# jkworldchampion/Video-Depth-Anything

Hardware: AMD Instinct MI355X
Metric: frames/sec at 1x32x518x518 fp16, ViT-L (higher is better)
Workload: dtype f16; 1 GPU; vitl fp16 32-frame clip forward, x=randn(1,32,3,518,518), seeded random weights (BASELINE.json configs[2]); parallelism=independent windows x1, world=1

## Files before the change

### video_depth_anything_amd/csrc/gemm.hip

```cpp
#include "gemm_epilogue.h"

namespace {
using vda_gemm::store_one;

constexpr int BK = 64;
constexpr int ROW_BYTES = BK * 2;
constexpr int NWAVES = 4;
constexpr int NTHREADS = NWAVES * 64;

template <int BM, int BN, int AMODE>
__global__ void __launch_bounds__(NTHREADS) gemm_kernel(const vda_gemm_args p) {
    constexpr int WTM = BM / 2, WTN = BN / 2;
    constexpr int MI = WTM / 16, NI = WTN / 16;
    constexpr int AJ = BM / 8 / NWAVES;
    constexpr int WJ = BN / 8 / NWAVES;
    constexpr int A_BYTES = BM * ROW_BYTES, W_BYTES = BN * ROW_BYTES, STAGE = A_BYTES + W_BYTES;

    extern __shared__ __attribute__((aligned(16))) char smem[];

    const int tid = threadIdx.x, lane = tid & 63;
    const int wave = __builtin_amdgcn_readfirstlane(tid >> 6);
    const int wm = wave >> 1, wn = wave & 1;

    const int nbn = (p.N + BN - 1) / BN;
    const int nwg = gridDim.x;
    const int bid = blockIdx.x;
    const int xcd = bid & 7, q = nwg >> 3, r = nwg & 7;
    const int t = (xcd < r ? xcd * (q + 1) : r * (q + 1) + (xcd - r) * q) + (bid >> 3);
    const int bm = t / nbn, bn = t - bm * nbn;
    const int m0 = bm * BM, n0 = bn * BN;

    const int lrow = lane >> 3;
    const int lchk = ((lane & 7) ^ lrow) * 8;
    const h16* a_src[AJ];
    int a_pix[AJ], a_iy0[AJ], a_ix0[AJ];
    const h16* w_src[WJ];
#pragma unroll
    for (int j = 0; j < AJ; ++j) {
        int m = m0 + (wave + NWAVES * j) * 8 + lrow;
        if constexpr (AMODE == VDA_A_DENSE) {
            m = min(m, p.M - 1);
            a_src[j] = (const h16*)p.A + (size_t)m * p.lda + lchk;
        } else {
            const bool ok = m < p.M;
            m = min(m, p.M - 1);
            const int hw = p.cHo * p.cWo;
            const int b = m / hw, rem = m - b * hw;
            const int oy = rem / p.cWo, ox = rem - oy * p.cWo;
            a_pix[j] = b * p.cH * p.cW;
            a_iy0[j] = ok ? oy * p.cStride - 1 : -100000;
            a_ix0[j] = ox * p.cStride - 1;
            a_src[j] = (const h16*)p.A + lchk;
        }
    }
#pragma unroll
    for (int j = 0; j < WJ; ++j) {
        const int n = min(n0 + (wave + NWAVES * j) * 8 + lrow, p.N - 1);
        w_src[j] = (const h16*)p.W + (size_t)n * p.K + lchk;
    }

    auto stage = [&](int kt, char* buf) {
        const int k0 = kt * BK;
        if constexpr (AMODE == VDA_A_DENSE) {
#pragma unroll
            for (int j = 0; j < AJ; ++j) glds16(a_src[j] + k0, buf + (wave + NWAVES * j) * 1024);
        } else {
            const int tap = k0 / p.cCin, ci0 = k0 - tap * p.cCin;
            const int ky = tap / 3, kx = tap - ky * 3;
#pragma unroll
            for (int j = 0; j < AJ; ++j) {
                const int iy = a_iy0[j] + ky, ix = a_ix0[j] + kx;
                const bool ok = (unsigned)iy < (unsigned)p.cH && (unsigned)ix < (unsigned)p.cW;
                const h16* src = ok ? a_src[j] + ((size_t)(a_pix[j] + iy * p.cW + ix) * p.cCin + ci0)
                                    : (const h16*)p.zero_page + lchk;
                glds16(src, buf + (wave + NWAVES * j) * 1024);
            }
        }
#pragma unroll
        for (int j = 0; j < WJ; ++j) glds16(w_src[j] + k0, buf + A_BYTES + (wave + NWAVES * j) * 1024);
    };

    f32x4 acc[MI][NI];
#pragma unroll
    for (int i = 0; i < MI; ++i)
#pragma unroll
        for (int j = 0; j < NI; ++j) acc[i][j] = f32x4{0.f, 0.f, 0.f, 0.f};

    const int frow = lane & 15, fchk = lane >> 4, fsw = lane & 7;
    const h16 relu_floor = p.relu_in ? (h16)0.f : (h16)(-65504.f);
    h16x8 relu_thr;
#pragma unroll
    for (int e = 0; e < 8; ++e) relu_thr[e] = relu_floor;

    auto compute = [&](const char* buf) {
        const char* At = buf + (wm * WTM + frow) * ROW_BYTES;
        const char* Wt = buf + A_BYTES + (wn * WTN + frow) * ROW_BYTES;
#pragma unroll
        for (int ks = 0; ks < 2; ++ks) {
            const int coff = ((ks * 4 + fchk) ^ fsw) << 4;
            h16x8 af[MI], wf[NI];
#pragma unroll
            for (int i = 0; i < MI; ++i) af[i] = *reinterpret_cast<const h16x8*>(At + i * 16 * ROW_BYTES + coff);
#pragma unroll
            for (int j = 0; j < NI; ++j) wf[j] = *reinterpret_cast<const h16x8*>(Wt + j * 16 * ROW_BYTES + coff);
            if constexpr (AMODE == VDA_A_CONV3X3) {
#pragma unroll
                for (int i = 0; i < MI; ++i) af[i] = __builtin_elementwise_max(af[i], relu_thr);
            }
#pragma unroll
            for (int i = 0; i < MI; ++i)
#pragma unroll
                for (int j = 0; j < NI; ++j)
                    acc[i][j] = __builtin_amdgcn_mfma_f32_16x16x32_f16(wf[j], af[i], acc[i][j], 0, 0, 0);
        }
    };

    const int nt = p.K / BK;
    stage(0, smem);
    asm volatile("s_waitcnt vmcnt(0)" ::: "memory");
    __syncthreads();
    int cur = 0;
    for (int kt = 0; kt < nt; ++kt) {
        if (kt + 1 < nt) stage(kt + 1, smem + (cur ^ 1) * STAGE);
        compute(smem + cur * STAGE);
        asm volatile("s_waitcnt vmcnt(0)" ::: "memory");
        __syncthreads();
        cur ^= 1;
    }

    const int em = m0 + wm * WTM + (lane & 15);
    const int en = n0 + wn * WTN + (lane >> 4) * 4;
    auto run = [&](auto epi_tag) {
        constexpr int EPI = decltype(epi_tag)::value;
        if constexpr (EPI == VDA_EPI_GEGLU_F16) {
#pragma unroll
            for (int i = 0; i < MI; ++i)
#pragma unroll
                for (int j = 0; j < NI; j += 2) store_one<EPI>(p, em + i * 16, en + j * 16, acc[i][j], acc[i][j + 1]);
        } else {
#pragma unroll
            for (int i = 0; i < MI; ++i)
#pragma unroll
                for (int j = 0; j < NI; ++j) store_one<EPI>(p, em + i * 16, en + j * 16, acc[i][j], acc[i][j]);
        }
    };
    vda_gemm::dispatch_epilogue(p.epilogue, run);
}

template <int BM, int BN, int AMODE>
int launch(const vda_gemm_args& a, hipStream_t s) {
    constexpr int smem = 2 * (BM + BN) * ROW_BYTES;
    static VdaKernelDeviceState dev_state;
    if (vda_prepare_kernel(reinterpret_cast<const void*>(&gemm_kernel<BM, BN, AMODE>), smem, dev_state) < 0) return 2;
    const int nbm = (a.M + BM - 1) / BM, nbn = (a.N + BN - 1) / BN;
    hipLaunchKernelGGL((gemm_kernel<BM, BN, AMODE>), dim3(nbm * nbn), dim3(NTHREADS), smem, s, a);
    VDA_LAUNCH_CHECK();
    return 0;
}

__global__ void __launch_bounds__(256) split_partials_kernel(const h16* __restrict__ hi, const h16* __restrict__ lo, float* __restrict__ part,
                                                             int M, int N, int ldc, int ld) {
    const int np = N >> 6;
    const long long i = (long long)blockIdx.x * 256 + threadIdx.x;
    if (i >= (long long)M * np) return;
    const int m = (int)(i / np), j = (int)(i - (long long)m * np);
    const h16* a = hi + (size_t)m * ldc + j * 64;
    const h16* b = lo + (size_t)m * ldc + j * 64;
    float sum = 0.f;
    for (int e = 0; e < 64; ++e) sum += (float)a[e] + (float)b[e];
    const float mean = sum * (1.f / 64.f);
    float sq = 0.f;
    for (int e = 0; e < 64; ++e) {
        const float d = ((float)a[e] + (float)b[e]) - mean;
        sq = fmaf(d, d, sq);
    }
    part[2 * ((size_t)j * ld + m)] = sum;
    part[2 * ((size_t)j * ld + m) + 1] = sq;
}

}

int vda_gemm256_dense_bn256(const vda_gemm_args& a, hipStream_t s);
int vda_gemm256_dense_bn128(const vda_gemm_args& a, hipStream_t s);
int vda_gemm256_conv_bn256(const vda_gemm_args& a, hipStream_t s);
int vda_gemm256_conv_bn128(const vda_gemm_args& a, hipStream_t s);
int vda_gemm256s_dense_bn256(const vda_gemm_args& a, hipStream_t s);
int vda_gemm256s_dense_bn128(const vda_gemm_args& a, hipStream_t s);
int vda_gemm256s_conv_bn256(const vda_gemm_args& a, hipStream_t s);
int vda_gemm256s_conv_bn128(const vda_gemm_args& a, hipStream_t s);
int vda_gemm256s_dense_bn128_bm192(const vda_gemm_args& a, hipStream_t s);
int vda_gemm256s_dense_bn128_bm192_x2(const vda_gemm_args& a, hipStream_t s);
int vda_gemm256s_dense_bn384_bm192(const vda_gemm_args& a, hipStream_t s);

int vda_gemm8p_dense_bn256(const vda_gemm_args& a, hipStream_t s);
int vda_gemm8p_conv_bn256(const vda_gemm_args& a, hipStream_t s);
int vda_gemm8p_dense_bn256_sched(const vda_gemm_args& a, hipStream_t s, int sched);
int vda_gemm8p_dense_bn128(const vda_gemm_args& a, hipStream_t s);
int vda_gemm8p_dense_bn256_bm192(const vda_gemm_args& a, hipStream_t s);
int vda_gemm8p_conv_bn128(const vda_gemm_args& a, hipStream_t s);

int vda_conv3x3_lds(const vda_gemm_args& a, hipStream_t s);

static int vda_gemm256s_launch(const vda_gemm_args& a, int bn, hipStream_t s) {
    if (a.a_mode == VDA_A_DENSE) return bn == 256 ? vda_gemm256s_dense_bn256(a, s) : vda_gemm256s_dense_bn128(a, s);
    return bn == 256 ? vda_gemm256s_conv_bn256(a, s) : vda_gemm256s_conv_bn128(a, s);
}

static int vda_gemm256_launch(const vda_gemm_args& a, int bn, hipStream_t s) {
    if (a.a_mode == VDA_A_DENSE) return bn == 256 ? vda_gemm256_dense_bn256(a, s) : vda_gemm256_dense_bn128(a, s);
    return bn == 256 ? vda_gemm256_conv_bn256(a, s) : vda_gemm256_conv_bn128(a, s);
}

static int launch_small(const vda_gemm_args& a, hipStream_t s) {
    const bool narrow = a.N <= 64;
    if (a.a_mode == VDA_A_DENSE) {
        const int rc = narrow ? launch<128, 64, VDA_A_DENSE>(a, s) : launch<128, 128, VDA_A_DENSE>(a, s);
        if (rc == 0 && a.epilogue == VDA_EPI_SCALE_RES_SPLIT) {
            const long long items = (long long)a.M * (a.N >> 6);
            hipLaunchKernelGGL(split_partials_kernel, dim3((unsigned)((items + 255) / 256)), dim3(256), 0, s, (const h16*)a.out, (const h16*)a.out2, a.stats, a.M,
                               a.N, a.ldc, a.stats_ld ? a.stats_ld : a.M);
            VDA_LAUNCH_CHECK();
        }
        return rc;
    }
    return narrow ? launch<128, 64, VDA_A_CONV3X3>(a, s) : launch<128, 128, VDA_A_CONV3X3>(a, s);
}

static int g_gemm_variant = -1;

static thread_local const char* g_last_kernel = "";

extern "C" const char* vda_gemm_last_kernel(void) { return g_last_kernel; }

extern "C" int vda_gemm_set_variant(int v) {
    g_gemm_variant = v;
    return 0;
}

static int g_gemm_debug = 0;

extern "C" int vda_gemm_set_debug(int flags) {
    g_gemm_debug = flags & 0xff;
    return 0;
}

static int device_cus() {
    static thread_local int ncu = 0;
    if (ncu == 0) {
        int dev = 0, cu = 0;
        (void)hipGetDevice(&dev);
        (void)hipDeviceGetAttribute(&cu, hipDeviceAttributeMultiprocessorCount, dev);
        ncu = cu < 8 ? 8 : (cu & ~7);
    }
    const int cap = g_vda_max_wgs;
    return (cap >= 8 && cap < ncu) ? (cap & ~7) : ncu;
}

static bool bm192_epilogue(int epilogue) {
    return epilogue == VDA_EPI_BIAS_F16 || epilogue == VDA_EPI_SCALE_RES_F32 || epilogue == VDA_EPI_SCALE_RES_SPLIT || epilogue == VDA_EPI_LN_BIAS_F16;
}

extern "C" int vda_gemm_plan_split(int M, int N, int K, int epilogue, int a_mode) {
    static const int allow = getenv("VDA_GEMM_SPLIT") ? atoi(getenv("VDA_GEMM_SPLIT")) : 1;
    static const int r192 = getenv("VDA_GEMM_R192") ? atoi(getenv("VDA_GEMM_R192")) : 84;
    if (!allow || a_mode != VDA_A_DENSE || !bm192_epilogue(epilogue) || M < 4096 || N < 256 || K < (allow == 2 ? 256 : 2048)) return M;
    const long long ncu = device_cus(), nbn = (N + 255) / 256;
    const long long rt = (M + 255) / 256;
    auto rounds = [&](long long tiles) { return (tiles + ncu - 1) / ncu; };
    const double t = 1.6 * (K / 64) + 5.0, launch = allow == 2 ? 0.0 : 10.0;
    const double single = (double)rounds(rt * nbn) * t;
    double best = single * 0.985;
    int best_m1 = M;
    for (long long r = 8; r * 256 < M; ++r) {
        const long long m2 = M - r * 256;
        if (m2 < 2048) break;
        const double cost = (double)rounds(r * nbn) * t + 0.01 * r192 * (double)rounds(((m2 + 191) / 192) * nbn) * t + launch;
        if (cost < best) {
            best = cost;
            best_m1 = (int)(r * 256);
        }
    }
    return best_m1;
}

static vda_gemm_args row_range(const vda_gemm_args& a0, int r0, int rows) {
    vda_gemm_args a = a0;
    if (a.lda == 0) a.lda = a.K;
    if (a.ldc == 0) a.ldc = a.N;
    vda_gemm_args p = a;
    auto adv = [&](const void* q, size_t bytes_per_row) -> const void* { return q ? (const char*)q + (size_t)r0 * bytes_per_row : nullptr; };
    const bool f32_out = a.epilogue == VDA_EPI_SCALE_RES_F32;
    const size_t ob = f32_out ? 4 : 2;
    p.A = adv(a.A, (size_t)a.lda * 2);
    p.out = const_cast<void*>(adv(a.out, (size_t)a.ldc * ob));
    if (a.epilogue == VDA_EPI_SCALE_RES_F32) p.res = adv(a.res, (size_t)a.ldc * 4);
    if (a.epilogue == VDA_EPI_SCALE_RES_SPLIT) {
        p.res = adv(a.res, (size_t)a.ldc * 2);
        p.res2 = adv(a.res2, (size_t)a.ldc * 2);
        p.out2 = const_cast<void*>(adv(a.out2, (size_t)a.ldc * 2));
        p.stats = (float*)const_cast<void*>(adv(a.stats, 8));
        p.stats_ld = a.stats_ld ? a.stats_ld : a.M;
        if (a.pos != nullptr && (const void*)a.pos != a.zero_page) p.pos = (const float*)adv(a.pos, 8);
    }
    if (a.epilogue == VDA_EPI_LN_BIAS_F16) p.stats = (float*)const_cast<void*>(adv(a.stats, 8));
    p.M = rows;
    return p;
}

extern "C" int vda_gemm_row_range(const vda_gemm_args* args, int r0, int rows, vda_gemm_args* out) {
    VDA_REQUIRE(args && out && r0 >= 0 && rows > 0 && r0 + rows <= args->M, "vda_gemm_row_range: bad range");
    VDA_REQUIRE(args->a_mode == VDA_A_DENSE && bm192_epilogue(args->epilogue), "vda_gemm_row_range: dense A and a row-splittable epilogue only");
    *out = row_range(*args, r0, rows);
    return 0;
}

static int vda_gemm_f16_impl(const vda_gemm_args* args, vda_stream_t stream, bool may_split);

extern "C" int vda_gemm_f16(const vda_gemm_args* args, vda_stream_t stream) { return vda_gemm_f16_impl(args, stream, true); }

static int vda_gemm_f16_impl(const vda_gemm_args* args, vda_stream_t stream, bool may_split) {
    VDA_REQUIRE(args != nullptr, "vda_gemm_f16: null args");
    vda_gemm_args a = *args;
    VDA_REQUIRE(a.A && a.W && a.out, "vda_gemm_f16: null operand");
    VDA_REQUIRE(a.M > 0 && a.N > 0 && a.K > 0, "vda_gemm_f16: empty problem M=%d N=%d K=%d", a.M, a.N, a.K);
    VDA_REQUIRE(a.K % BK == 0, "vda_gemm_f16: K=%d must be a multiple of %d (pad at pack time)", a.K, BK);
    VDA_REQUIRE(a.N % 4 == 0 && a.ldc % 4 == 0, "vda_gemm_f16: N=%d and ldc=%d must be multiples of 4", a.N, a.ldc);
    VDA_REQUIRE(((uintptr_t)a.A & 15) == 0 && ((uintptr_t)a.W & 15) == 0 && ((uintptr_t)a.out & 15) == 0,
                "vda_gemm_f16: operands must be 16-byte aligned");
    VDA_REQUIRE(a.epilogue >= 0 && a.epilogue <= VDA_EPI_LN_GELU_F16, "vda_gemm_f16: bad epilogue %d", a.epilogue);
    if (a.a_mode == VDA_A_DENSE) {
        VDA_REQUIRE(a.relu_in == 0, "vda_gemm_f16: relu_in is only built for the conv A operand");
        VDA_REQUIRE((a.lda >= a.K || a.lda == 0) && a.lda % 8 == 0, "vda_gemm_f16: lda=%d must be >= K (or 0 = broadcast row) and a multiple of 8", a.lda);
    } else if (a.a_mode == VDA_A_CONV3X3) {
        VDA_REQUIRE(a.zero_page != nullptr, "vda_gemm_f16: conv needs zero_page");
        VDA_REQUIRE(a.cCin % BK == 0 && a.K == 9 * a.cCin, "vda_gemm_f16: conv needs Cin%%64==0 and K==9*Cin (Cin=%d K=%d)", a.cCin, a.K);
        VDA_REQUIRE(a.cStride == 1 || a.cStride == 2, "vda_gemm_f16: conv stride %d", a.cStride);
        VDA_REQUIRE(a.cHo == (a.cH + 2 - 3) / a.cStride + 1 && a.cWo == (a.cW + 2 - 3) / a.cStride + 1,
                    "vda_gemm_f16: conv output size mismatch");
        VDA_REQUIRE(a.M == a.cB * a.cHo * a.cWo, "vda_gemm_f16: conv M=%d != B*Ho*Wo", a.M);
        VDA_REQUIRE((long long)a.cB * a.cH * a.cW * a.cCin < (1ll << 31), "vda_gemm_f16: conv input too large for 32-bit pixel index");
    } else {
        VDA_REQUIRE(false, "vda_gemm_f16: bad a_mode %d", a.a_mode);
    }
    switch (a.epilogue) {
        case VDA_EPI_SCALE_RES_F32:
        case VDA_EPI_SCALE_RES_F32_H:
        case VDA_EPI_RES_F16:
            VDA_REQUIRE(a.res != nullptr, "vda_gemm_f16: residual epilogue needs res");
            break;
        case VDA_EPI_GEGLU_F16:
            VDA_REQUIRE(a.N % 32 == 0, "vda_gemm_f16: GEGLU needs N%%32==0");
            break;
        case VDA_EPI_SCALE_RES_SPLIT:
            VDA_REQUIRE(a.res != nullptr && a.res2 != nullptr && a.out2 != nullptr && a.stats != nullptr,
                        "vda_gemm_f16: the split-residual epilogue needs res, res2 (hi / lo planes), out2 and stats");
            VDA_REQUIRE(a.N % 64 == 0 && a.ldc % 8 == 0 && a.a_mode == VDA_A_DENSE, "vda_gemm_f16: the split-residual epilogue needs a dense A operand, N%%64==0 and ldc%%8==0");
            VDA_REQUIRE(((uintptr_t)a.res & 15) == 0 && ((uintptr_t)a.res2 & 15) == 0 && ((uintptr_t)a.out2 & 15) == 0 && ((uintptr_t)a.stats & 7) == 0,
                        "vda_gemm_f16: split-residual planes must be 16-byte aligned");
            if (a.pos != nullptr && (const void*)a.pos != a.zero_page) {
                VDA_REQUIRE(((uintptr_t)a.pos & 7) == 0, "vda_gemm_f16: pos (re-centring statistics) must be 8-byte aligned");
                a.P = 2;
            } else {
                VDA_REQUIRE(a.zero_page != nullptr, "vda_gemm_f16: the split-residual epilogue without pos needs zero_page");
                a.pos = (const float*)a.zero_page;
                a.P = 0;
            }
            break;
        case VDA_EPI_LN_BIAS_F16:
        case VDA_EPI_LN_GELU_F16:
            VDA_REQUIRE(a.stats != nullptr && a.gamma != nullptr && a.bias != nullptr && a.a_mode == VDA_A_DENSE,
                        "vda_gemm_f16: a LayerNorm-folded epilogue needs a dense A operand, stats (mean, rstd rows), gamma (= c1) and bias (= c2)");
            VDA_REQUIRE(((uintptr_t)a.stats & 7) == 0, "vda_gemm_f16: stats must be 8-byte aligned");
            break;
        case VDA_EPI_PATCH_F32:
            VDA_REQUIRE(a.pos != nullptr && a.P > 0 && a.M % a.P == 0, "vda_gemm_f16: patch epilogue needs pos and M%%P==0");
            break;
        case VDA_EPI_CONVT_F16:
            VDA_REQUIRE(a.tK > 0 && a.tCout > 0 && a.tCout % 4 == 0 && a.N == a.tK * a.tK * a.tCout && a.M % (a.tH * a.tW) == 0,
                        "vda_gemm_f16: bad ConvTranspose geometry");
            break;
        default:
            break;
    }
    hipStream_t s = (hipStream_t)stream;
    static const int conv_lds = getenv("VDA_CONV_LDS") ? atoi(getenv("VDA_CONV_LDS")) : 1;
    if (a.a_mode == VDA_A_CONV3X3 && ((g_gemm_variant < 0 && conv_lds) || g_gemm_variant == 7)) {
        const int rc = vda_conv3x3_lds(a, s);
        if (rc >= 0) {
            g_last_kernel = a.N <= 32 ? "conv3x3_lds_kernel<1>" : "conv3x3_lds_kernel<2>";
            return rc;
        }
    }
    const bool fits32 = (a.a_mode == VDA_A_DENSE ? (long long)a.M * a.lda : 0ll) + a.K < (1ll << 31) && (long long)a.N * a.K < (1ll << 31);
    VDA_REQUIRE(fits32 || g_gemm_variant == 0 || g_gemm_variant < 0, "vda_gemm_f16: operand too large for the 256-row kernel's 32-bit offsets");
    if (!fits32) return launch_small(a, s);
    int big = 0, small_mfma = 1;
    bool eight = g_gemm_variant >= 5 && (g_gemm_variant & 15) == 5;
    if (eight) big = 256;
    if (g_gemm_variant == 1 || g_gemm_variant == 3) big = 256;
    if (g_gemm_variant == 2 || g_gemm_variant == 4 || g_gemm_variant == 8 || g_gemm_variant == 10 || g_gemm_variant == 11) big = 128;
    if (g_gemm_variant == 1 || g_gemm_variant == 2) small_mfma = 0;
    if (g_gemm_variant == 9) {
        eight = true;
        big = 128;
    }
    static const int big_min_n = getenv("VDA_GEMM_BIG_MIN_N") ? atoi(getenv("VDA_GEMM_BIG_MIN_N")) : 192;
    if (g_gemm_variant < 0 && a.N >= big_min_n && a.M >= 2048) {
        const int pad256 = (a.N + 255) / 256 * 256, pad128 = (a.N + 127) / 128 * 128;
        big = pad128 < pad256 ? 128 : 256;
        static const int eight128 = getenv("VDA_GEMM_8P128") ? atoi(getenv("VDA_GEMM_8P128")) : 0;
        if (big == 256 || eight128) eight = true;
    }
    if (big && (a.N % 8 != 0 || a.ldc % 8 != 0)) {
        VDA_REQUIRE(g_gemm_variant < 0, "vda_gemm_f16: the 256-row kernel needs N and ldc to be multiples of 8");
        big = 0;
    }
    if (big) {
        vda_gemm_args a8 = a;
        static const int stagger = getenv("VDA_GEMM_STAGGER") ? atoi(getenv("VDA_GEMM_STAGGER")) : 0;
        if (!stagger) a8.relu_in |= 16 << 8;
        if (stagger == 2) a8.relu_in |= 32 << 8;
        if (eight && g_gemm_variant > 0) a8.relu_in = (a.relu_in & 0xff) | (((g_gemm_variant >> 4) & 0xff) << 8);
        a8.relu_in |= g_gemm_debug << 16;
        static const long long nt_mb = getenv("VDA_GEMM_NT_MB") ? atoll(getenv("VDA_GEMM_NT_MB")) : 192;
        if (nt_mb > 0 && (long long)a.M * a.N * 2 >= nt_mb * 1000000ll) a8.relu_in |= 1 << 24;
        const int sched8 = (eight && g_gemm_variant > 0) ? ((g_gemm_variant >> 5) & 3) : 0;
        bool tall192 = g_gemm_variant == 8 && a.a_mode == VDA_A_DENSE;
        const int ncu = device_cus();
        if (g_gemm_variant < 0 && !eight && big == 128 && a.a_mode == VDA_A_DENSE) {
            const long long nbn = (a.N + 127) / 128;
            const long long r256 = (((a.M + 255) / 256) * nbn + ncu - 1) / ncu, r192 = (((a.M + 191) / 192) * nbn + ncu - 1) / ncu;
            static const int allow192 = getenv("VDA_GEMM_BM192") ? atoi(getenv("VDA_GEMM_BM192")) : 1;
            tall192 = allow192 && r192 * 3 * 100 < r256 * 4 * 85;
        }
        static const int small_grid = getenv("VDA_GEMM_SMALL_GRID") ? atoi(getenv("VDA_GEMM_SMALL_GRID")) : 1;
        if (g_gemm_variant < 0 && small_grid && ((long long)(a.M + 255) / 256) * ((a.N + big - 1) / big) * 2 <= ncu) {
            g_last_kernel = a.a_mode == VDA_A_DENSE ? (a.N <= 64 ? "gemm_kernel<128, 64, 0>" : "gemm_kernel<128, 128, 0>")
                                                    : (a.N <= 64 ? "gemm_kernel<128, 64, 1>" : "gemm_kernel<128, 128, 1>");
            return launch_small(a, s);
        }
        static const int wide384 = getenv("VDA_GEMM_BN384") ? atoi(getenv("VDA_GEMM_BN384")) : 2;
        const bool ln_epi = a.epilogue == VDA_EPI_LN_BIAS_F16 || a.epilogue == VDA_EPI_LN_GELU_F16;
        const bool auto384 = g_gemm_variant < 0 && a.tile_rows == 0 &&
                             (wide384 == 1 ? (!eight && a.N <= 1152)
                                            : wide384 == 2 ? ((a.N == 384 && a.K >= 1024) || (ln_epi && a.N <= 1536))
                                            : wide384 == 3 ? (a.N == 384 && a.K >= 1024)
                                            : wide384 == 4 ? ((a.N == 384 && a.K >= 1024) || (ln_epi && a.N == 1536)) : false);
        if (a.a_mode == VDA_A_DENSE && a.N % 384 == 0 && (auto384 || g_gemm_variant == 10)) {
            const int rc384 = vda_gemm256s_dense_bn384_bm192(a8, s);
            if (rc384 >= 0) {
                static thread_local char name384[64];
                snprintf(name384, sizeof(name384), "gemm256s_kernel<384, %d, %d, 192, 1>", a.a_mode, a.epilogue);
                g_last_kernel = name384;
                return rc384;
            }
        }
        if (eight && big == 256 && a.a_mode == VDA_A_DENSE && g_gemm_variant < 0 && may_split && a.tile_rows == 0 && a.sched == nullptr && a.lda != 0) {
            const int m1 = vda_gemm_plan_split(a.M, a.N, a.K, a.epilogue, a.a_mode);
            if (m1 < a.M) {
                vda_gemm_args p1 = row_range(a, 0, m1), p2 = row_range(a, m1, a.M - m1);
                p2.tile_rows = 192;
                const int rc1 = vda_gemm_f16_impl(&p1, stream, false);
                if (rc1 != 0) return rc1;
                return vda_gemm_f16_impl(&p2, stream, false);
            }
        }
        if (eight && big == 256 && a.a_mode == VDA_A_DENSE && (a.tile_rows == 192 || g_gemm_variant == 5 + 16 * 64)) {
            const int rc192 = vda_gemm8p_dense_bn256_bm192(a8, s);
            if (rc192 >= 0) {
                static thread_local char name192[64];
                snprintf(name192, sizeof(name192), "gemm8p_kernel<256, %d, %d, 1, 192, %s>", a.a_mode, a.epilogue, a.sched ? "true" : "false");
                g_last_kernel = name192;
                return rc192;
            }
        }
        if (g_gemm_variant == 11 && a.a_mode == VDA_A_DENSE) {
            const int rcx2 = vda_gemm256s_dense_bn128_bm192_x2(a8, s);
            if (rcx2 >= 0) {
                static thread_local char namex2[64];
                snprintf(namex2, sizeof(namex2), "gemm256s_kernel<128, %d, %d, 192, 2>", a.a_mode, a.epilogue);
                g_last_kernel = namex2;
                return rcx2;
            }
        }
        if (tall192) {
            const int rc192 = vda_gemm256s_dense_bn128_bm192(a8, s);
            if (rc192 >= 0) {
                static thread_local char name192[64];
                snprintf(name192, sizeof(name192), "gemm256s_kernel<128, %d, %d, 192, 1>", a.a_mode, a.epilogue);
                g_last_kernel = name192;
                return rc192;
            }
        }
        const int rc = !eight ? (small_mfma ? vda_gemm256s_launch(a8, big, s) : vda_gemm256_launch(a, big, s))
                       : big == 128 ? (a.a_mode == VDA_A_DENSE ? vda_gemm8p_dense_bn128(a8, s) : vda_gemm8p_conv_bn128(a8, s))
                       : a.a_mode == VDA_A_DENSE ? (sched8 ? vda_gemm8p_dense_bn256_sched(a8, s, sched8) : vda_gemm8p_dense_bn256(a8, s))
                                                 : vda_gemm8p_conv_bn256(a8, s);
        if (rc >= 0) {
            static thread_local char name[64];
            const int sch = sched8 == 1 ? 0 : sched8 == 2 ? 2 : 1;
            if (eight) snprintf(name, sizeof(name), "gemm8p_kernel<%d, %d, %d, %d, 256, %s>", big, a.a_mode, a.epilogue, sch, (a.sched && sch == 1) ? "true" : "false");
            else if (small_mfma) snprintf(name, sizeof(name), "gemm256s_kernel<%d, %d, %d, 256, 1>", big, a.a_mode, a.epilogue);
            else snprintf(name, sizeof(name), "gemm256_kernel<%d, %d, %d>", big, a.a_mode, a.epilogue);
            g_last_kernel = name;
            return rc;
        }
    }
    g_last_kernel = a.a_mode == VDA_A_DENSE ? (a.N <= 64 ? "gemm_kernel<128, 64, 0>" : "gemm_kernel<128, 128, 0>")
                                            : (a.N <= 64 ? "gemm_kernel<128, 64, 1>" : "gemm_kernel<128, 128, 1>");
    return launch_small(a, s);
}
```

### video_depth_anything_amd/csrc/host.hip

```cpp
#include "vda_common.h"
#include <string.h>
#include <exception>
#include <type_traits>
#include <array>
#include <map>
#include <string>
#include <vector>

namespace {

constexpr int PATCH = 14, POS_GRID = 37, KPATCH = 640, GN_GROUPS = 32, TEMPORAL_HEADS = 8;
constexpr float ENC_LN_EPS = 1e-6f, GN_EPS = 1e-6f, TMP_LN_EPS = 1e-5f;

inline int pad64(int c) { return (c + 63) / 64 * 64; }

#define VDA_TRY(expr)            \
    do {                         \
        const int rc_ = (expr);  \
        if (rc_ != 0) return rc_; \
    } while (0)

#define VDA_HIP(expr)                                                      \
    do {                                                                   \
        const hipError_t e_ = (expr);                                      \
        if (e_ != hipSuccess) {                                            \
            vda_set_error("%s: %s", #expr, hipGetErrorString(e_));         \
            return 2;                                                      \
        }                                                                  \
    } while (0)

template <typename T>
__global__ void pack_matrix_kernel(const float* __restrict__ src, T* __restrict__ dst, int N, int K, int Npad, int Kpad) {
    const size_t total = (size_t)Npad * Kpad;
    for (size_t i = (size_t)blockIdx.x * 256 + threadIdx.x; i < total; i += (size_t)gridDim.x * 256) {
        const int n = (int)(i / Kpad), k = (int)(i - (size_t)n * Kpad);
        dst[i] = (n < N && k < K) ? (T)src[(size_t)n * K + k] : (T)0.f;
    }
}
template <typename T>
__global__ void pack_conv3x3_kernel(const float* __restrict__ src, T* __restrict__ dst, int Co, int Ci, int Copad, int Cipad) {
    const size_t total = (size_t)Copad * 9 * Cipad;
    for (size_t i = (size_t)blockIdx.x * 256 + threadIdx.x; i < total; i += (size_t)gridDim.x * 256) {
        const int ci = (int)(i % Cipad);
        const size_t t = i / Cipad;
        const int tap = (int)(t % 9), co = (int)(t / 9);
        dst[i] = (co < Co && ci < Ci) ? (T)src[((size_t)co * Ci + ci) * 9 + tap] : (T)0.f;
    }
}
template <typename T>
__global__ void pack_convt_kernel(const float* __restrict__ src, T* __restrict__ dst, int Ci, int Co, int k, int cpad) {
    const size_t total = (size_t)k * k * cpad * cpad;
    for (size_t i = (size_t)blockIdx.x * 256 + threadIdx.x; i < total; i += (size_t)gridDim.x * 256) {
        const int ci = (int)(i % cpad);
        const size_t t = i / cpad;
        const int co = (int)(t % cpad), tap = (int)(t / cpad);
        dst[i] = (co < Co && ci < Ci) ? (T)src[((size_t)ci * Co + co) * k * k + tap] : (T)0.f;
    }
}
__global__ void expand_convt_bias_kernel(const float* __restrict__ b, float* __restrict__ dst, int Co, int kk, int cpad) {
    const int i = blockIdx.x * 256 + threadIdx.x;
    if (i >= kk * cpad) return;
    const int co = i % cpad;
    dst[i] = co < Co ? b[co] : 0.f;
}
template <typename T>
__global__ void pack_geglu_kernel(const float* __restrict__ src, T* __restrict__ dst, int n, int K) {
    const size_t total = (size_t)2 * n * K;
    for (size_t i = (size_t)blockIdx.x * 256 + threadIdx.x; i < total; i += (size_t)gridDim.x * 256) {
        const int R = (int)(i / K), k = (int)(i - (size_t)R * K);
        const int blk = R >> 5, within = R & 31;
        const int srow = within < 16 ? blk * 16 + within : n + blk * 16 + (within - 16);
        dst[i] = (T)src[(size_t)srow * K + k];
    }
}

inline unsigned grid_for(size_t items) {
    const size_t b = (items + 255) / 256;
    return (unsigned)(b < 1 ? 1 : (b > 65535 ? 65535 : b));
}

#ifndef VDA_LN_FOLD_DEFAULT
#define VDA_LN_FOLD_DEFAULT 1
#endif

__global__ void __launch_bounds__(256) poison_on_overflow_kernel(const int* __restrict__ flag, float* __restrict__ depth, long long n,
                                                                 volatile int* __restrict__ host_report) {
    if (*flag == 0) return;
    for (long long i = (long long)blockIdx.x * 256 + threadIdx.x; i < n; i += (long long)gridDim.x * 256) depth[i] = __builtin_nanf("");
    if (blockIdx.x == 0 && threadIdx.x == 0) {
        *host_report = 1;
        __threadfence_system();
    }
}

struct Raw {
    float* d = nullptr;
    std::vector<int64_t> dims;
    size_t n = 0;
};

struct ProfSample {
    std::string name;
    double flops;
    hipEvent_t e0, e1;
};
struct Profile {
    int every = 0;
    double min_flops = 0.0;
    std::map<std::array<int, 5>, int> seen;
    std::map<std::string, std::pair<long long, double>> launches;
    std::vector<ProfSample> samples;
};

struct Layout {
    int gemm_launches = 0;
    std::map<std::string, std::pair<size_t, size_t>> bufs;
    std::vector<std::string> order;
    size_t total = 0;
};

}

struct vda_model {
    vda_config cfg;
    int device = 0;
    std::map<std::string, std::vector<int64_t>> spec;
    std::map<std::string, Raw> raw;
    std::map<std::string, void*> mat[2];
    std::map<std::string, float*> vec;
    bool finalized = false, packed[2] = {false, false};
    float oc3_bias = 0.f;
    void* zero_page = nullptr;
    std::map<std::pair<int, int>, float*> pos_cache;
    void* ws = nullptr;
    int64_t ws_bytes = 0;
    bool ws_owned = false;
    std::map<std::array<int, 5>, Layout> layouts;
    std::vector<void*> owned;
    int ocp[4] = {0, 0, 0, 0}, Fhp = 0;
    std::array<int, 5> last_key = {0, 0, 0, 0, -1};
    Profile prof;
    int residual_in_ln = 0;
    int dyn_sched = 0;
    int ln_fold = VDA_LN_FOLD_DEFAULT;
    int oc1_fused = 1;
    int head_overlap = 0;
    struct Side {
        hipStream_t stream = nullptr;
        hipEvent_t fork = nullptr, join = nullptr;
    };
    std::map<hipStream_t, Side> sides;
    int mlp_fused = 0;
    volatile int32_t* ovf_host = nullptr;
};

namespace {

using Spec = std::map<std::string, std::vector<int64_t>>;

void build_spec(const vda_config& c, Spec& s) {
    const int64_t D = c.embed_dim, F = c.features;
    const int64_t oc[4] = {c.out_channels[0], c.out_channels[1], c.out_channels[2], c.out_channels[3]};
    auto put = [&](const std::string& k, std::vector<int64_t> v) { s[k] = std::move(v); };
    const std::string p = "pretrained.";
    put(p + "cls_token", {1, 1, D});
    put(p + "pos_embed", {1, POS_GRID * POS_GRID + 1, D});
    put(p + "mask_token", {1, D});
    put(p + "patch_embed.proj.weight", {D, 3, PATCH, PATCH});
    put(p + "patch_embed.proj.bias", {D});
    for (int i = 0; i < c.depth; ++i) {
        const std::string b = p + "blocks." + std::to_string(i) + ".";
        put(b + "norm1.weight", {D});
        put(b + "norm1.bias", {D});
        put(b + "attn.qkv.weight", {3 * D, D});
        put(b + "attn.qkv.bias", {3 * D});
        put(b + "attn.proj.weight", {D, D});
        put(b + "attn.proj.bias", {D});
        put(b + "ls1.gamma", {D});
        put(b + "norm2.weight", {D});
        put(b + "norm2.bias", {D});
        put(b + "mlp.fc1.weight", {4 * D, D});
        put(b + "mlp.fc1.bias", {4 * D});
        put(b + "mlp.fc2.weight", {D, 4 * D});
        put(b + "mlp.fc2.bias", {D});
        put(b + "ls2.gamma", {D});
    }
    put(p + "norm.weight", {D});
    put(p + "norm.bias", {D});
    const std::string h = "head.";
    for (int i = 0; i < 4; ++i) {
        put(h + "projects." + std::to_string(i) + ".weight", {oc[i], D, 1, 1});
        put(h + "projects." + std::to_string(i) + ".bias", {oc[i]});
    }
    put(h + "resize_layers.0.weight", {oc[0], oc[0], 4, 4});
    put(h + "resize_layers.0.bias", {oc[0]});
    put(h + "resize_layers.1.weight", {oc[1], oc[1], 2, 2});
    put(h + "resize_layers.1.bias", {oc[1]});
    put(h + "resize_layers.3.weight", {oc[3], oc[3], 3, 3});
    put(h + "resize_layers.3.bias", {oc[3]});
    if (c.use_clstoken)
        for (int i = 0; i < 4; ++i) {
            put(h + "readout_projects." + std::to_string(i) + ".0.weight", {D, 2 * D});
            put(h + "readout_projects." + std::to_string(i) + ".0.bias", {D});
        }
    const std::string sc = h + "scratch.";
    for (int i = 0; i < 4; ++i) put(sc + "layer" + std::to_string(i + 1) + "_rn.weight", {F, oc[i], 3, 3});
    for (int i = 1; i <= 4; ++i) {
        const std::string r = sc + "refinenet" + std::to_string(i) + ".";
        put(r + "out_conv.weight", {F, F, 1, 1});
        put(r + "out_conv.bias", {F});
        for (int u = 1; u <= 2; ++u)
            for (int cc = 1; cc <= 2; ++cc) {
                const std::string k = r + "resConfUnit" + std::to_string(u) + ".conv" + std::to_string(cc);
                put(k + ".weight", {F, F, 3, 3});
                put(k + ".bias", {F});
            }
        if (c.use_bn)
            for (int u = 1; u <= 2; ++u)
                for (int cc = 1; cc <= 2; ++cc) {
                    const std::string k = r + "resConfUnit" + std::to_string(u) + ".bn" + std::to_string(cc) + ".";
                    put(k + "weight", {F});
                    put(k + "bias", {F});
                    put(k + "running_mean", {F});
                    put(k + "running_var", {F});
                    put(k + "num_batches_tracked", {});
                }
    }
    put(sc + "output_conv1.weight", {F / 2, F, 3, 3});
    put(sc + "output_conv1.bias", {F / 2});
    put(sc + "output_conv2.0.weight", {32, F / 2, 3, 3});
    put(sc + "output_conv2.0.bias", {32});
    put(sc + "output_conv2.2.weight", {1, 32, 1, 1});
    put(sc + "output_conv2.2.bias", {1});
    const int64_t tc[4] = {oc[2], oc[3], F, F};
    for (int m = 0; m < 4; ++m) {
        const int64_t C = tc[m];
        const std::string t = h + "motion_modules." + std::to_string(m) + ".temporal_transformer.";
        put(t + "norm.weight", {C});
        put(t + "norm.bias", {C});
        put(t + "proj_in.weight", {C, C});
        put(t + "proj_in.bias", {C});
        const std::string tb = t + "transformer_blocks.0.";
        for (int a = 0; a < 2; ++a) {
            const std::string ab = tb + "attention_blocks." + std::to_string(a) + ".";
            put(ab + "to_q.weight", {C, C});
            put(ab + "to_k.weight", {C, C});
            put(ab + "to_v.weight", {C, C});
            put(ab + "to_out.0.weight", {C, C});
            put(ab + "to_out.0.bias", {C});
            if (!c.pe_rope) put(ab + "pos_encoder.pe", {1, c.num_frames, C});
            put(tb + "norms." + std::to_string(a) + ".weight", {C});
            put(tb + "norms." + std::to_string(a) + ".bias", {C});
        }
        put(tb + "ff.net.0.proj.weight", {8 * C, C});
        put(tb + "ff.net.0.proj.bias", {8 * C});
        put(tb + "ff.net.2.weight", {C, 4 * C});
        put(tb + "ff.net.2.bias", {C});
        put(tb + "ff_norm.weight", {C});
        put(tb + "ff_norm.bias", {C});
        put(t + "proj_out.weight", {C, C});
        put(t + "proj_out.bias", {C});
    }
}

int dev_alloc(vda_model* h, size_t bytes, void** out) {
    void* p = nullptr;
    VDA_HIP(hipMalloc(&p, bytes < 256 ? 256 : bytes));
    h->owned.push_back(p);
    *out = p;
    return 0;
}

int require_device(const vda_model* h, const char* what) {
    int dev = -1;
    VDA_HIP(hipGetDevice(&dev));
    if (dev != h->device) {
        vda_set_error("%s: the handle lives on device %d but device %d is current (one handle per device; make it current)", what, h->device, dev);
        return 1;
    }
    return 0;
}

__global__ void __launch_bounds__(256) fold_bn_kernel(const float* __restrict__ W, const float* __restrict__ b, const float* __restrict__ g,
                                                      const float* __restrict__ beta, const float* __restrict__ rm, const float* __restrict__ rv,
                                                      float* __restrict__ Wo, float* __restrict__ bo, int Co, int per_co) {
    const long long n = (long long)Co * per_co;
    for (long long i = (long long)blockIdx.x * 256 + threadIdx.x; i < n; i += (long long)gridDim.x * 256) {
        const int co = (int)(i / per_co);
        const float sc = g[co] / sqrtf(rv[co] + 1e-5f);
        Wo[i] = W[i] * sc;
        if (i - (long long)co * per_co == 0) bo[co] = (b[co] - rm[co]) * sc + beta[co];
    }
}

template <typename T>
int pack_all(vda_model* h, int prec) {
    const vda_config& c = h->cfg;
    hipStream_t s = nullptr;
    auto raw = [&](const std::string& k) -> const float* { return h->raw.at(k).d; };
    auto mat = [&](const std::string& key, size_t elems, T** out) -> int {
        void* p = nullptr;
        VDA_TRY(dev_alloc(h, elems * sizeof(T), &p));
        h->mat[prec][key] = p;
        *out = (T*)p;
        return 0;
    };
    auto lin = [&](const std::string& key, const std::string& name, int N, int K, int Npad, int Kpad) -> int {
        T* d = nullptr;
        VDA_TRY(mat(key, (size_t)Npad * Kpad, &d));
        hipLaunchKernelGGL((pack_matrix_kernel<T>), dim3(grid_for((size_t)Npad * Kpad)), dim3(256), 0, s, raw(name), d, N, K, Npad, Kpad);
        return 0;
    };
    auto conv = [&](const std::string& key, const std::string& name, int Co, int Ci, int Copad, int Cipad) -> int {
        T* d = nullptr;
        VDA_TRY(mat(key, (size_t)Copad * 9 * Cipad, &d));
        hipLaunchKernelGGL((pack_conv3x3_kernel<T>), dim3(grid_for((size_t)Copad * 9 * Cipad)), dim3(256), 0, s, raw(name), d, Co, Ci, Copad, Cipad);
        return 0;
    };
    const bool vecs = h->vec.empty();
    auto vecp = [&](const std::string& key, const std::string& name, int n, int npad) -> int {
        if (!vecs) return 0;
        void* p = nullptr;
        VDA_TRY(dev_alloc(h, (size_t)npad * sizeof(float), &p));
        h->vec[key] = (float*)p;
        hipLaunchKernelGGL((pack_matrix_kernel<float>), dim3(grid_for(npad)), dim3(256), 0, s, raw(name), (float*)p, 1, n, 1, npad);
        return 0;
    };
    const int D = c.embed_dim, Fe = c.features;
    const int* oc = c.out_channels;
    const int* ocp = h->ocp;
    const int Fh = Fe / 2, Fhp = h->Fhp;
    const std::string p = "pretrained.";
    VDA_TRY(lin("patch.w", p + "patch_embed.proj.weight", D, 588, D, KPATCH));
    VDA_TRY(vecp("patch.b", p + "patch_embed.proj.bias", D, D));
    VDA_TRY(vecp("cls", p + "cls_token", D, D));
    for (int i = 0; i < c.depth; ++i) {
        const std::string b = p + "blocks." + std::to_string(i) + ".", k = "b" + std::to_string(i) + ".";
        VDA_TRY(vecp(k + "norm1.weight", b + "norm1.weight", D, D));
        VDA_TRY(vecp(k + "norm1.bias", b + "norm1.bias", D, D));
        VDA_TRY(vecp(k + "norm2.weight", b + "norm2.weight", D, D));
        VDA_TRY(vecp(k + "norm2.bias", b + "norm2.bias", D, D));
        VDA_TRY(vecp(k + "attn.qkv.bias", b + "attn.qkv.bias", 3 * D, 3 * D));
        VDA_TRY(vecp(k + "attn.proj.bias", b + "attn.proj.bias", D, D));
        VDA_TRY(vecp(k + "mlp.fc1.bias", b + "mlp.fc1.bias", 4 * D, 4 * D));
        VDA_TRY(vecp(k + "mlp.fc2.bias", b + "mlp.fc2.bias", D, D));
        VDA_TRY(vecp(k + "ls1.gamma", b + "ls1.gamma", D, D));
        VDA_TRY(vecp(k + "ls2.gamma", b + "ls2.gamma", D, D));
        VDA_TRY(lin(k + "attn.qkv.weight", b + "attn.qkv.weight", 3 * D, D, 3 * D, D));
        VDA_TRY(lin(k + "attn.proj.weight", b + "attn.proj.weight", D, D, D, D));
        VDA_TRY(lin(k + "mlp.fc1.weight", b + "mlp.fc1.weight", 4 * D, D, 4 * D, D));
        VDA_TRY(lin(k + "mlp.fc2.weight", b + "mlp.fc2.weight", D, 4 * D, D, 4 * D));
        if constexpr (std::is_same<T, h16>::value) {
            const char* pairs[2][3] = {{"attn.qkv", "norm1", nullptr}, {"mlp.fc1", "norm2", nullptr}};
            const int outs[2] = {3 * D, 4 * D};
            for (int j = 0; j < 2; ++j) {
                const std::string lk = pairs[j][0], nk = pairs[j][1];
                T* d = nullptr;
                VDA_TRY(mat(k + lk + ".weight.ln", (size_t)outs[j] * D, &d));
                void *c1 = nullptr, *c2 = nullptr;
                VDA_TRY(dev_alloc(h, (size_t)outs[j] * sizeof(float), &c1));
                VDA_TRY(dev_alloc(h, (size_t)outs[j] * sizeof(float), &c2));
                h->vec[k + lk + ".c1"] = (float*)c1;
                h->vec[k + lk + ".c2"] = (float*)c2;
                VDA_TRY(vda_fold_ln_weight(raw(b + lk + ".weight"), raw(b + lk + ".bias"), raw(b + nk + ".weight"), raw(b + nk + ".bias"), d, (float*)c1,
                                           (float*)c2, outs[j], D, s));
            }
            if (vda_mlp_fused_supported(D, 4 * D)) {
                T* d = nullptr;
                VDA_TRY(mat(k + "mlp.fc2.weight.perm", (size_t)D * 4 * D, &d));
                VDA_TRY(vda_mlp_permute_w2_f16(h->mat[prec].at(k + "mlp.fc2.weight"), d, D, 4 * D, s));
            }
        }
    }
    VDA_TRY(vecp("norm.w", p + "norm.weight", D, D));
    VDA_TRY(vecp("norm.b", p + "norm.bias", D, D));
    const std::string hd = "head.";
    if (c.use_clstoken)
        for (int i = 0; i < 4; ++i) {
            const std::string n = hd + "readout_projects." + std::to_string(i) + ".0", k = "readout" + std::to_string(i);
            VDA_TRY(lin(k + ".w", n + ".weight", D, 2 * D, D, 2 * D));
            VDA_TRY(vecp(k + ".b", n + ".bias", D, D));
        }
    for (int i = 0; i < 4; ++i) {
        const std::string n = hd + "projects." + std::to_string(i), k = "proj" + std::to_string(i);
        VDA_TRY(lin(k + ".w", n + ".weight", oc[i], D, ocp[i], D));
        VDA_TRY(vecp(k + ".b", n + ".bias", oc[i], ocp[i]));
    }
    for (int i = 0; i < 2; ++i) {
        const int kk = i == 0 ? 4 : 2, cp = ocp[i];
        const std::string n = hd + "resize_layers." + std::to_string(i), k = "resize" + std::to_string(i);
        T* d = nullptr;
        VDA_TRY(mat(k + ".w", (size_t)kk * kk * cp * cp, &d));
        hipLaunchKernelGGL((pack_convt_kernel<T>), dim3(grid_for((size_t)kk * kk * cp * cp)), dim3(256), 0, s, raw(n + ".weight"), d, oc[i], oc[i], kk, cp);
        if (vecs) {
            void* bp = nullptr;
            VDA_TRY(dev_alloc(h, (size_t)kk * kk * cp * sizeof(float), &bp));
            h->vec[k + ".b"] = (float*)bp;
            hipLaunchKernelGGL(expand_convt_bias_kernel, dim3((kk * kk * cp + 255) / 256), dim3(256), 0, s, raw(n + ".bias"), (float*)bp, oc[i], kk * kk, cp);
        }
    }
    VDA_TRY(conv("resize3.w", hd + "resize_layers.3.weight", oc[3], oc[3], ocp[3], ocp[3]));
    VDA_TRY(vecp("resize3.b", hd + "resize_layers.3.bias", oc[3], ocp[3]));
    const std::string sc = hd + "scratch.";
    for (int i = 0; i < 4; ++i)
        VDA_TRY(conv("rn" + std::to_string(i + 1) + ".w", sc + "layer" + std::to_string(i + 1) + "_rn.weight", Fe, oc[i], Fe, ocp[i]));
    for (int i = 1; i <= 4; ++i) {
        const std::string r = sc + "refinenet" + std::to_string(i) + ".", k = "ref" + std::to_string(i) + ".";
        VDA_TRY(lin(k + "out.w", r + "out_conv.weight", Fe, Fe, Fe, Fe));
        VDA_TRY(vecp(k + "out.b", r + "out_conv.bias", Fe, Fe));
        for (int u = 1; u <= 2; ++u)
            for (int cc = 1; cc <= 2; ++cc) {
                const std::string rn = r + "resConfUnit" + std::to_string(u) + ".conv" + std::to_string(cc);
                const std::string kn = k + "rcu" + std::to_string(u) + ".c" + std::to_string(cc);
                if (c.use_bn) {
                    const std::string bn = r + "resConfUnit" + std::to_string(u) + ".bn" + std::to_string(cc) + ".";
                    Raw& fw = h->raw[rn + ".weight.bn"];
                    Raw& fb = h->raw[rn + ".bias.bn"];
                    if (fw.d == nullptr) {
                        void *pw = nullptr, *pb = nullptr;
                        VDA_TRY(dev_alloc(h, (size_t)Fe * Fe * 9 * sizeof(float), &pw));
                        VDA_TRY(dev_alloc(h, (size_t)Fe * sizeof(float), &pb));
                        fw.d = (float*)pw, fw.n = (size_t)Fe * Fe * 9;
                        fb.d = (float*)pb, fb.n = Fe;
                    }
                    hipLaunchKernelGGL(fold_bn_kernel, dim3(grid_for((size_t)Fe * Fe * 9)), dim3(256), 0, s, raw(rn + ".weight"), raw(rn + ".bias"), raw(bn + "weight"),
                                       raw(bn + "bias"), raw(bn + "running_mean"), raw(bn + "running_var"), fw.d, fb.d, Fe, Fe * 9);
                    VDA_TRY(conv(kn + ".w", rn + ".weight.bn", Fe, Fe, Fe, Fe));
                    VDA_TRY(vecp(kn + ".b", rn + ".bias.bn", Fe, Fe));
                    continue;
                }
                VDA_TRY(conv(kn + ".w", rn + ".weight", Fe, Fe, Fe, Fe));
                VDA_TRY(vecp(kn + ".b", rn + ".bias", Fe, Fe));
            }
    }
    VDA_TRY(conv("oc1.w", sc + "output_conv1.weight", Fh, Fe, Fhp, Fe));
    VDA_TRY(vecp("oc1.b", sc + "output_conv1.bias", Fh, Fhp));
    VDA_TRY(conv("oc2.w", sc + "output_conv2.0.weight", 32, Fh, 32, Fhp));
    VDA_TRY(vecp("oc2.b", sc + "output_conv2.0.bias", 32, 32));
    VDA_TRY(vecp("oc3.w", sc + "output_conv2.2.weight", 32, 32));
    const int tc[4] = {ocp[2], ocp[3], Fe, Fe};
    for (int m = 0; m < 4; ++m) {
        const int Cc = tc[m];
        const std::string t = hd + "motion_modules." + std::to_string(m) + ".temporal_transformer.", k = "tm" + std::to_string(m) + ".";
        VDA_TRY(vecp(k + "gn.w", t + "norm.weight", Cc, Cc));
        VDA_TRY(vecp(k + "gn.b", t + "norm.bias", Cc, Cc));
        VDA_TRY(lin(k + "in.w", t + "proj_in.weight", Cc, Cc, Cc, Cc));
        VDA_TRY(vecp(k + "in.b", t + "proj_in.bias", Cc, Cc));
        VDA_TRY(lin(k + "out.w", t + "proj_out.weight", Cc, Cc, Cc, Cc));
        VDA_TRY(vecp(k + "out.b", t + "proj_out.bias", Cc, Cc));
        const std::string tb = t + "transformer_blocks.0.";
        for (int a = 0; a < 2; ++a) {
            const std::string ab = tb + "attention_blocks." + std::to_string(a) + ".", ka = k + "a" + std::to_string(a) + ".";
            T* d = nullptr;
            VDA_TRY(mat(ka + "qkv.w", (size_t)3 * Cc * Cc, &d));
            const char* names[3] = {"to_q.weight", "to_k.weight", "to_v.weight"};
            for (int j = 0; j < 3; ++j)
                hipLaunchKernelGGL((pack_matrix_kernel<T>), dim3(grid_for((size_t)Cc * Cc)), dim3(256), 0, s, raw(ab + names[j]),
                                   d + (size_t)j * Cc * Cc, Cc, Cc, Cc, Cc);
            VDA_TRY(lin(ka + "out.w", ab + "to_out.0.weight", Cc, Cc, Cc, Cc));
            VDA_TRY(vecp(ka + "out.b", ab + "to_out.0.bias", Cc, Cc));
            if (!c.pe_rope) VDA_TRY(vecp(ka + "pe", ab + "pos_encoder.pe", c.num_frames * Cc, c.num_frames * Cc));
            VDA_TRY(vecp(ka + "ln.w", tb + "norms." + std::to_string(a) + ".weight", Cc, Cc));
            VDA_TRY(vecp(ka + "ln.b", tb + "norms." + std::to_string(a) + ".bias", Cc, Cc));
        }
        VDA_TRY(vecp(k + "ffln.w", tb + "ff_norm.weight", Cc, Cc));
        VDA_TRY(vecp(k + "ffln.b", tb + "ff_norm.bias", Cc, Cc));
        {
            T* d = nullptr;
            VDA_TRY(mat(k + "ff1.w", (size_t)8 * Cc * Cc, &d));
            hipLaunchKernelGGL((pack_geglu_kernel<T>), dim3(grid_for((size_t)8 * Cc * Cc)), dim3(256), 0, s, raw(tb + "ff.net.0.proj.weight"), d, 4 * Cc, Cc);
            if (vecs) {
                void* bp = nullptr;
                VDA_TRY(dev_alloc(h, (size_t)8 * Cc * sizeof(float), &bp));
                h->vec[k + "ff1.b"] = (float*)bp;
                hipLaunchKernelGGL((pack_geglu_kernel<float>), dim3(grid_for((size_t)8 * Cc)), dim3(256), 0, s, raw(tb + "ff.net.0.proj.bias"), (float*)bp, 4 * Cc, 1);
            }
        }
        VDA_TRY(lin(k + "ff2.w", tb + "ff.net.2.weight", Cc, 4 * Cc, Cc, 4 * Cc));
        VDA_TRY(vecp(k + "ff2.b", tb + "ff.net.2.bias", Cc, Cc));
    }
    VDA_HIP(hipGetLastError());
    VDA_HIP(hipStreamSynchronize(s));
    h->packed[prec] = true;
    return 0;
}

struct Run {
    vda_model* h;
    int prec;
    bool dry;
    Layout* lay;
    hipStream_t s;
    size_t ab;
    int32_t* sched = nullptr;
    int nsched = 0;

    void* buf(const std::string& name, size_t elems, size_t esize) {
        const size_t bytes = (elems * esize + 255) & ~(size_t)255;
        if (dry) {
            auto it = lay->bufs.find(name);
            if (it == lay->bufs.end()) {
                lay->bufs[name] = {0, bytes};
                lay->order.push_back(name);
            } else if (it->second.second < bytes) {
                it->second.second = bytes;
            }
            return (void*)(uintptr_t)256;
        }
        return (char*)h->ws + lay->bufs.at(name).first;
    }
    void* act(const std::string& name, size_t elems) { return buf(name, elems, ab); }
    float* f32(const std::string& name, size_t elems) { return (float*)buf(name, elems, 4); }
    const void* W(const std::string& k) const { return dry ? nullptr : h->mat[prec].at(k); }
    const float* V(const std::string& k) const { return dry ? nullptr : h->vec.at(k); }

    int gemm(vda_gemm_args a) {
        if (prec == VDA_PREC_F16) {
            const int m1 = vda_gemm_plan_split(a.M, a.N, a.K, a.epilogue, a.a_mode);
            if (m1 < a.M) {
                if (dry) {
                    VDA_TRY(gemm_one(a));
                    return gemm_one(a);
                }
                vda_gemm_args p1, p2;
                a.zero_page = h->zero_page;
                VDA_TRY(vda_gemm_row_range(&a, 0, m1, &p1));
                VDA_TRY(vda_gemm_row_range(&a, m1, a.M - m1, &p2));
                p1.tile_rows = 256;
                p2.tile_rows = 192;
                VDA_TRY(gemm_one(p1));
                return gemm_one(p2);
            }
        }
        return gemm_one(a);
    }
    int gemm_one(vda_gemm_args a) {
        if (prec == VDA_PREC_F16 && h->dyn_sched) {
            if (!dry && sched != nullptr) a.sched = sched + 8 * nsched;
            ++nsched;
        }
        if (dry) return 0;
        a.zero_page = h->zero_page;
        if (a.lda == 0) a.lda = a.K;
        if (a.ldc == 0) a.ldc = a.N;
        Profile& pf = h->prof;
        if (pf.every <= 0) return prec == VDA_PREC_F32 ? vda_gemm_f32(&a, s) : vda_gemm_f16(&a, s);
        const std::array<int, 5> key = {a.M, a.N, a.K, a.epilogue, a.a_mode};
        const int n = pf.seen[key]++;
        const bool timed = n % pf.every == 0 && 2.0 * a.M * a.N * a.K >= pf.min_flops;
        ProfSample smp;
        if (timed) {
            VDA_HIP(hipEventCreate(&smp.e0));
            VDA_HIP(hipEventCreate(&smp.e1));
            VDA_HIP(hipEventRecord(smp.e0, s));
        }
        VDA_TRY(prec == VDA_PREC_F32 ? vda_gemm_f32(&a, s) : vda_gemm_f16(&a, s));
        const std::string name = prec == VDA_PREC_F32 ? std::string("gemm_f32_kernel") : std::string(vda_gemm_last_kernel());
        const double flops = 2.0 * a.M * a.N * a.K;
        auto& tot = pf.launches[name];
        tot.first += 1;
        tot.second += flops;
        if (timed) {
            VDA_HIP(hipEventRecord(smp.e1, s));
            smp.name = name;
            smp.flops = flops;
            pf.samples.push_back(smp);
        }
        return 0;
    }
    int dense(const void* A, const void* Wm, void* out, int epi, int M, int N, int K, const float* bias = nullptr, const void* res = nullptr,
              const float* gamma = nullptr, int ldc = 0) {
        vda_gemm_args a = {};
        a.A = A, a.W = Wm, a.out = out, a.bias = bias, a.res = res, a.gamma = gamma;
        a.M = M, a.N = N, a.K = K, a.ldc = ldc, a.a_mode = VDA_A_DENSE, a.epilogue = epi;
        return gemm(a);
    }
    int conv3x3(const void* x, const std::string& wname, void* out, int B, int H, int Wd, int Cin, int Cout, int epi, int stride,
                const float* bias, bool relu_in = false, const void* res = nullptr, const void* res2 = nullptr) {
        const int Ho = (H - 1) / stride + 1, Wo = (Wd - 1) / stride + 1;
        vda_gemm_args a = {};
        a.A = x, a.W = W(wname), a.out = out, a.bias = bias, a.res = res, a.res2 = res2;
        a.M = B * Ho * Wo, a.N = Cout, a.K = 9 * Cin, a.a_mode = VDA_A_CONV3X3, a.epilogue = epi, a.relu_in = relu_in ? 1 : 0;
        a.cB = B, a.cH = H, a.cW = Wd, a.cCin = Cin, a.cHo = Ho, a.cWo = Wo, a.cStride = stride;
        return gemm(a);
    }
    int layernorm(const float* x, void* out, const float* w, const float* b, float eps, int rows, int D, int group = 0, int skip = 0,
                  const float* pe = nullptr, int pe_rows = 0, int pe_steps = 0) {
        if (dry) return 0;
        return prec == VDA_PREC_F32 ? vda_layernorm_f32_f32(x, (float*)out, w, b, eps, rows, D, group, skip, pe, pe_rows, pe_steps, s)
                                    : vda_layernorm_f32_f16(x, out, w, b, eps, rows, D, group, skip, pe, pe_rows, pe_steps, s);
    }
    int bilinear(const void* x, void* out, int B, int hh, int ww, int H, int Wd, int C) {
        if (dry) return 0;
        return prec == VDA_PREC_F32 ? vda_bilinear_nhwc_f32((const float*)x, (float*)out, nullptr, B, hh, ww, H, Wd, C, s)
                                    : vda_bilinear_nhwc_f16(x, out, nullptr, B, hh, ww, H, Wd, C, s);
    }

    int temporal(int m, const void* x, int B, int T, int hw, int Cc, const std::string& tag, void** result) {
        const std::string k = "tm" + std::to_string(m) + ".";
        const int BT = B * T, rows = BT * hw;
        int chunks = (hw + 31) / 32;
        chunks = chunks < 1 ? 1 : (chunks > 16 ? 16 : chunks);
        float* part = f32("gn_partial", (size_t)BT * chunks * GN_GROUPS * 2);
        void* g = act("tm_g", (size_t)rows * Cc);
        if (!dry)
            VDA_TRY(prec == VDA_PREC_F32 ? vda_groupnorm_nhwc_f32((const float*)x, (float*)g, V(k + "gn.w"), V(k + "gn.b"), GN_EPS, BT, hw, Cc, GN_GROUPS, part, chunks, s)
                                         : vda_groupnorm_nhwc_f16(x, g, V(k + "gn.w"), V(k + "gn.b"), GN_EPS, BT, hw, Cc, GN_GROUPS, part, chunks, s));
        float* hs = f32("tm_hs", (size_t)rows * Cc);
        VDA_TRY(dense(g, W(k + "in.w"), hs, VDA_EPI_BIAS_F32, rows, Cc, Cc, V(k + "in.b")));
        void* n = act("tm_n", (size_t)rows * Cc);
        void* qkv = act("tm_qkv", (size_t)rows * 3 * Cc);
        void* ao = act("tm_ao", (size_t)rows * Cc);
        for (int a = 0; a < 2; ++a) {
            const std::string ka = k + "a" + std::to_string(a) + ".";
            const bool rope = h->cfg.pe_rope != 0;
            VDA_TRY(layernorm(hs, n, V(ka + "ln.w"), V(ka + "ln.b"), TMP_LN_EPS, rows, Cc, 0, 0, rope ? nullptr : V(ka + "pe"), hw, T));
            VDA_TRY(dense(n, W(ka + "qkv.w"), qkv, VDA_EPI_BIAS_F16, rows, 3 * Cc, Cc));
            for (int b = 0; b < B && !dry; ++b) {
                const size_t r0 = (size_t)b * T * hw;
                if (rope)
                    VDA_TRY(prec == VDA_PREC_F32 ? vda_rope_qk_f32((float*)qkv + r0 * 3 * Cc, T, hw, Cc, s) : vda_rope_qk_f16((h16*)qkv + r0 * 3 * Cc, T, hw, Cc, s));
                VDA_TRY(prec == VDA_PREC_F32
                            ? vda_temporal_attention_f32((const float*)qkv + r0 * 3 * Cc, (float*)ao + r0 * Cc, T, hw, Cc, TEMPORAL_HEADS, s)
                            : vda_temporal_attention_f16((const h16*)qkv + r0 * 3 * Cc, (h16*)ao + r0 * Cc, T, hw, Cc, TEMPORAL_HEADS, s));
            }
            VDA_TRY(dense(ao, W(ka + "out.w"), hs, VDA_EPI_SCALE_RES_F32, rows, Cc, Cc, V(ka + "out.b"), hs));
        }
        VDA_TRY(layernorm(hs, n, V(k + "ffln.w"), V(k + "ffln.b"), TMP_LN_EPS, rows, Cc));
        void* gg = act("tm_gg", (size_t)rows * 4 * Cc);
        VDA_TRY(dense(n, W(k + "ff1.w"), gg, VDA_EPI_GEGLU_F16, rows, 8 * Cc, Cc, V(k + "ff1.b"), nullptr, nullptr, 4 * Cc));
        void* hh = act("tm_hh", (size_t)rows * Cc);
        VDA_TRY(dense(gg, W(k + "ff2.w"), hh, VDA_EPI_SCALE_RES_F32_H, rows, Cc, 4 * Cc, V(k + "ff2.b"), hs));
        void* out = act(tag, (size_t)rows * Cc);
        VDA_TRY(dense(hh, W(k + "out.w"), out, VDA_EPI_RES_F16, rows, Cc, Cc, V(k + "out.b"), x));
        *result = out;
        return 0;
    }

    int rcu(int i, int u, const void* x, void* out, int B, int H, int Wd, int Fe, const void* res2 = nullptr) {
        const std::string k = "ref" + std::to_string(i) + ".rcu" + std::to_string(u) + ".";
        void* y = act("rcu_y", (size_t)B * H * Wd * Fe);
        VDA_TRY(conv3x3(x, k + "c1.w", y, B, H, Wd, Fe, Fe, VDA_EPI_BIAS_RELU_F16, 1, V(k + "c1.b"), true));
        VDA_TRY(conv3x3(y, k + "c2.w", out, B, H, Wd, Fe, Fe, VDA_EPI_RES_F16, 1, V(k + "c2.b"), false, x, res2));
        return 0;
    }
    int fusion(int i, const void* x0, const void* x1, int B, int H, int Wd, int Ho, int Wo, int Fe, const std::string& tag, void** result,
               bool upsample = true) {
        const size_t rows = (size_t)B * H * Wd;
        const void* sm = x0;
        if (x1 != nullptr) {
            void* t = act("fus_s", rows * Fe);
            VDA_TRY(rcu(i, 1, x1, t, B, H, Wd, Fe, x0));
            sm = t;
        }
        void* r = act("fus_r", rows * Fe);
        VDA_TRY(rcu(i, 2, sm, r, B, H, Wd, Fe));
        void* c = act(upsample ? "fus_c" : tag, rows * Fe);
        const std::string k = "ref" + std::to_string(i) + ".out.";
        VDA_TRY(dense(r, W(k + "w"), c, VDA_EPI_BIAS_F16, (int)rows, Fe, Fe, V(k + "b")));
        if (!upsample) {
            *result = c;
            return 0;
        }
        void* out = act(tag, (size_t)B * Ho * Wo * Fe);
        VDA_TRY(bilinear(c, out, B, H, Wd, Ho, Wo, Fe));
        *result = out;
        return 0;
    }

    int forward(const float* x, float* depth, int B, int T, int H, int Wd) {
        const vda_config& c = h->cfg;
        const int BT = B * T, ph = H / PATCH, pw = Wd / PATCH;
        const int P = ph * pw, D = c.embed_dim, NH = c.num_heads, Nt = P + 1, rows = BT * Nt;
        if (prec == VDA_PREC_F16 && h->dyn_sched) {
            const int cap = dry ? 4096 : lay->gemm_launches;
            sched = (int32_t*)buf("sched", (size_t)8 * (cap > 0 ? cap : 1), 4);
            if (!dry) VDA_HIP(hipMemsetAsync(sched, 0, (size_t)32 * lay->gemm_launches, s));
            nsched = 0;
        }
        void* a0 = act("a0", (size_t)BT * P * KPATCH);
        if (!dry) {
            VDA_HIP(hipMemsetAsync(a0, 0, (size_t)BT * P * KPATCH * ab, s));
            VDA_TRY(prec == VDA_PREC_F32 ? vda_patchify_f32_f32(x, (float*)a0, BT, H, Wd, KPATCH, s) : vda_patchify_f32_f16(x, a0, BT, H, Wd, KPATCH, s));
        }
        float* tok = f32("tok", (size_t)rows * D);
        const float* pos = dry ? nullptr : h->pos_cache.at({H, Wd});
        {
            vda_gemm_args a = {};
            a.A = a0, a.W = W("patch.w"), a.out = tok, a.bias = V("patch.b"), a.pos = pos;
            a.M = BT * P, a.N = D, a.K = KPATCH, a.a_mode = VDA_A_DENSE, a.epilogue = VDA_EPI_PATCH_F32, a.P = P;
            VDA_TRY(gemm(a));
        }
        if (!dry) VDA_TRY(vda_cls_rows_f32(tok, V("cls"), pos, BT, P, D, s));
        void* xn = act("xn", (size_t)rows * D);
        void* qkv = act("qkv", (size_t)rows * 3 * D);
        void* ao = act("ao", (size_t)rows * D);
        void* hid = nullptr;
        void* taps[4] = {nullptr, nullptr, nullptr, nullptr};
        int ntap = 0;
        const bool defer = prec == VDA_PREC_F16 && h->residual_in_ln != 0;
        const bool fold = prec == VDA_PREC_F16 && h->ln_fold != 0 && !defer && D % 64 == 0;
        const bool mlp1 = fold && h->mlp_fused != 0 && vda_mlp_fused_supported(D, 4 * D) != 0;
        if (!mlp1) hid = act("hid", (size_t)rows * 4 * D);
        void* thi = fold ? buf("tok_hi", (size_t)rows * D, 2) : nullptr;
        void* tlo = fold ? buf("tok_lo", (size_t)rows * D, 2) : nullptr;
        float* lnpart = fold ? f32("ln_part", (size_t)rows * (D / 64) * 2) : nullptr;
        float* lnstat = fold ? f32("ln_stat", (size_t)rows * 2) : nullptr;
        int32_t* ovf = fold ? (int32_t*)buf("overflow", 1, 4) : nullptr;
        if (fold && !dry) VDA_HIP(hipMemsetAsync(ovf, 0, 4, s));
        if (fold && !dry) VDA_TRY(vda_split_center_stats_f32(tok, thi, tlo, lnstat, ENC_LN_EPS, rows, D, s));
        auto ln_gemm = [&](const std::string& wk, void* out, int epi, int N) -> int {
            vda_gemm_args a = {};
            a.A = thi, a.W = W(wk + ".weight.ln"), a.out = out, a.bias = V(wk + ".c2"), a.gamma = V(wk + ".c1"), a.stats = lnstat;
            a.M = rows, a.N = N, a.K = D, a.a_mode = VDA_A_DENSE, a.epilogue = epi;
            return gemm(a);
        };
        auto res_gemm = [&](const void* A, const std::string& wk, const std::string& gk, int K, bool stats_next) -> int {
            vda_gemm_args a = {};
            a.A = A, a.W = W(wk + ".weight"), a.out = thi, a.out2 = tlo, a.res = thi, a.res2 = tlo, a.bias = V(wk + ".bias"), a.gamma = V(gk);
            a.stats = lnpart;
            a.pos = lnstat;
            a.M = rows, a.N = D, a.K = K, a.a_mode = VDA_A_DENSE, a.epilogue = VDA_EPI_SCALE_RES_SPLIT;
            VDA_TRY(gemm(a));
            (void)stats_next;
            if (!dry) VDA_TRY(vda_ln_stats_finalize(lnpart, lnstat, ENC_LN_EPS, rows, D / 64, ovf, s));
            return 0;
        };
        auto tap_ln = [&](void* out, int group, int skip) -> int {
            if (dry) return 0;
            return fold ? vda_layernorm_split_f16(thi, tlo, out, V("norm.w"), V("norm.b"), ENC_LN_EPS, rows, D, group, skip, s)
                        : vda_layernorm_f32_f16(tok, out, V("norm.w"), V("norm.b"), ENC_LN_EPS, rows, D, group, skip, nullptr, 0, 0, s);
        };
        void* yb = defer ? act("ybuf", (size_t)rows * D) : nullptr;
        auto ln_res = [&](const float* gamma, void* out, const float* w, const float* b, int group, int skip) -> int {
            if (dry) return 0;
            return vda_layernorm_residual_f32_f16(tok, yb, gamma, out, w, b, ENC_LN_EPS, rows, D, group, skip, s);
        };
        bool xn_ready = false;
        const int* ocp = h->ocp;
        const int Fe = c.features, Fhp = h->Fhp;
        const int h1 = 4 * ph, w1 = 4 * pw, h2 = 2 * ph, w2 = 2 * pw, h4 = (ph - 1) / 2 + 1, w4 = (pw - 1) / 2 + 1;
        void *l1r = nullptr, *l2r = nullptr, *l3r = nullptr;
        auto head_early = [&]() -> int {
            void* t0 = act("t0", (size_t)BT * P * ocp[0]);
            VDA_TRY(dense(taps[0], W("proj0.w"), t0, VDA_EPI_BIAS_F16, BT * P, ocp[0], D, V("proj0.b")));
            void* l1 = act("l1", (size_t)BT * h1 * w1 * ocp[0]);
            {
                vda_gemm_args a = {};
                a.A = t0, a.W = W("resize0.w"), a.out = l1, a.bias = V("resize0.b");
                a.M = BT * P, a.N = 16 * ocp[0], a.K = ocp[0], a.ldc = ocp[0], a.a_mode = VDA_A_DENSE, a.epilogue = VDA_EPI_CONVT_F16;
                a.tK = 4, a.tH = ph, a.tW = pw, a.tCout = ocp[0];
                VDA_TRY(gemm(a));
            }
            void* t1 = act("t1", (size_t)BT * P * ocp[1]);
            VDA_TRY(dense(taps[1], W("proj1.w"), t1, VDA_EPI_BIAS_F16, BT * P, ocp[1], D, V("proj1.b")));
            void* l2 = act("l2", (size_t)BT * h2 * w2 * ocp[1]);
            {
                vda_gemm_args a = {};
                a.A = t1, a.W = W("resize1.w"), a.out = l2, a.bias = V("resize1.b");
                a.M = BT * P, a.N = 4 * ocp[1], a.K = ocp[1], a.ldc = ocp[1], a.a_mode = VDA_A_DENSE, a.epilogue = VDA_EPI_CONVT_F16;
                a.tK = 2, a.tH = ph, a.tW = pw, a.tCout = ocp[1];
                VDA_TRY(gemm(a));
            }
            void* l3 = act("l3", (size_t)BT * P * ocp[2]);
            VDA_TRY(dense(taps[2], W("proj2.w"), l3, VDA_EPI_BIAS_F16, BT * P, ocp[2], D, V("proj2.b")));
            void* l3t = nullptr;
            VDA_TRY(temporal(0, l3, B, T, P, ocp[2], "l3t", &l3t));
            l1r = act("l1r", (size_t)BT * h1 * w1 * Fe);
            VDA_TRY(conv3x3(l1, "rn1.w", l1r, BT, h1, w1, ocp[0], Fe, VDA_EPI_BIAS_F16, 1, nullptr));
            l2r = act("l2r", (size_t)BT * h2 * w2 * Fe);
            VDA_TRY(conv3x3(l2, "rn2.w", l2r, BT, h2, w2, ocp[1], Fe, VDA_EPI_BIAS_F16, 1, nullptr));
            l3r = act("l3r", (size_t)BT * P * Fe);
            VDA_TRY(conv3x3(l3t, "rn3.w", l3r, BT, ph, pw, ocp[2], Fe, VDA_EPI_BIAS_F16, 1, nullptr));
            return 0;
        };
        bool early_done = false;
        vda_model::Side* side = nullptr;
        for (int i = 0; i < c.depth; ++i) {
            const std::string k = "b" + std::to_string(i) + ".";
            if (fold) {
                VDA_TRY(ln_gemm(k + "attn.qkv", qkv, VDA_EPI_LN_BIAS_F16, 3 * D));
            } else {
                if (!xn_ready) VDA_TRY(layernorm(tok, xn, V(k + "norm1.weight"), V(k + "norm1.bias"), ENC_LN_EPS, rows, D));
                xn_ready = false;
                VDA_TRY(dense(xn, W(k + "attn.qkv.weight"), qkv, VDA_EPI_BIAS_F16, rows, 3 * D, D, V(k + "attn.qkv.bias")));
            }
            if (!dry) VDA_TRY(prec == VDA_PREC_F32 ? vda_attention_f32((const float*)qkv, (float*)ao, BT, Nt, NH, s) : vda_attention_f16(qkv, ao, BT, Nt, NH, s));
            if (fold) {
                VDA_TRY(res_gemm(ao, k + "attn.proj", k + "ls1.gamma", D, true));
            } else if (defer) {
                VDA_TRY(dense(ao, W(k + "attn.proj.weight"), yb, VDA_EPI_BIAS_F16, rows, D, D, V(k + "attn.proj.bias")));
                VDA_TRY(ln_res(V(k + "ls1.gamma"), xn, V(k + "norm2.weight"), V(k + "norm2.bias"), 0, 0));
            } else {
                VDA_TRY(dense(ao, W(k + "attn.proj.weight"), tok, VDA_EPI_SCALE_RES_F32, rows, D, D, V(k + "attn.proj.bias"), tok, V(k + "ls1.gamma")));
                VDA_TRY(layernorm(tok, xn, V(k + "norm2.weight"), V(k + "norm2.bias"), ENC_LN_EPS, rows, D));
            }
            if (mlp1) {
                if (!dry)
                    VDA_TRY(vda_mlp_fused_f16(thi, lnstat, W(k + "mlp.fc1.weight.ln"), V(k + "mlp.fc1.c1"), V(k + "mlp.fc1.c2"), W(k + "mlp.fc2.weight.perm"),
                                              V(k + "mlp.fc2.bias"), V(k + "ls2.gamma"), thi, tlo, lnpart, rows, D, 4 * D, rows, s));
            } else if (fold) VDA_TRY(ln_gemm(k + "mlp.fc1", hid, VDA_EPI_LN_GELU_F16, 4 * D));
            else VDA_TRY(dense(xn, W(k + "mlp.fc1.weight"), hid, VDA_EPI_BIAS_GELU_F16, rows, 4 * D, D, V(k + "mlp.fc1.bias")));
            bool is_tap = false;
            for (int t = 0; t < 4; ++t) is_tap = is_tap || c.taps[t] == i;
            const bool last = i + 1 == c.depth;
            void* tp = (is_tap && ntap < 4) ? act("tap" + std::to_string(ntap), (size_t)BT * P * D) : nullptr;
            if (fold) {
                if (mlp1) {
                    if (!dry) VDA_TRY(vda_ln_stats_finalize(lnpart, lnstat, ENC_LN_EPS, rows, D / 64, ovf, s));
                } else {
                    VDA_TRY(res_gemm(hid, k + "mlp.fc2", k + "ls2.gamma", 4 * D, !last));
                }
                if (tp != nullptr) VDA_TRY(tap_ln(tp, Nt, 1));
            } else if (defer) {
                VDA_TRY(dense(hid, W(k + "mlp.fc2.weight"), yb, VDA_EPI_BIAS_F16, rows, D, 4 * D, V(k + "mlp.fc2.bias")));
                if (last && tp != nullptr) {
                    VDA_TRY(ln_res(V(k + "ls2.gamma"), tp, V("norm.w"), V("norm.b"), Nt, 1));
                } else {
                    const std::string kn = "b" + std::to_string(last ? i : i + 1) + ".";
                    VDA_TRY(ln_res(V(k + "ls2.gamma"), xn, V(kn + "norm1.weight"), V(kn + "norm1.bias"), 0, 0));
                    xn_ready = true;
                    if (tp != nullptr) VDA_TRY(layernorm(tok, tp, V("norm.w"), V("norm.b"), ENC_LN_EPS, rows, D, Nt, 1));
                }
            } else {
                VDA_TRY(dense(hid, W(k + "mlp.fc2.weight"), tok, VDA_EPI_SCALE_RES_F32, rows, D, 4 * D, V(k + "mlp.fc2.bias"), tok, V(k + "ls2.gamma")));
                if (tp != nullptr) VDA_TRY(layernorm(tok, tp, V("norm.w"), V("norm.b"), ENC_LN_EPS, rows, D, Nt, 1));
            }
            if (tp != nullptr) {
                if (c.use_clstoken) {
                    void* full = act("rd_full", (size_t)rows * D);
                    VDA_TRY(fold ? tap_ln(full, 0, 0) : layernorm(tok, full, V("norm.w"), V("norm.b"), ENC_LN_EPS, rows, D));
                    void* cat = act("rd_cat", (size_t)BT * P * 2 * D);
                    if (!dry)
                        VDA_TRY(prec == VDA_PREC_F32 ? vda_readout_concat_f32((const float*)full, (float*)cat, BT, P, D, s)
                                                     : vda_readout_concat_f16(full, cat, BT, P, D, s));
                    const std::string kr = "readout" + std::to_string(ntap);
                    VDA_TRY(dense(cat, W(kr + ".w"), tp, VDA_EPI_BIAS_GELU_F16, BT * P, D, 2 * D, V(kr + ".b")));
                }
                taps[ntap++] = tp;
                if (ntap == 3 && !last && !early_done) {
                    if (dry || !h->head_overlap) {
                        if (dry) {
                            VDA_TRY(head_early());
                            early_done = true;
                        }
                    } else {
                        vda_model::Side& sd = h->sides[s];
                        if (sd.stream == nullptr) {
                            VDA_HIP(hipStreamCreateWithFlags(&sd.stream, hipStreamNonBlocking));
                            VDA_HIP(hipEventCreateWithFlags(&sd.fork, hipEventDisableTiming));
                            VDA_HIP(hipEventCreateWithFlags(&sd.join, hipEventDisableTiming));
                        }
                        side = &sd;
                        VDA_HIP(hipEventRecord(sd.fork, s));
                        VDA_HIP(hipStreamWaitEvent(sd.stream, sd.fork, 0));
                        hipStream_t main_stream = s;
                        s = sd.stream;
                        const int rc = head_early();
                        s = main_stream;
                        if (rc != 0) return rc;
                        VDA_HIP(hipEventRecord(sd.join, sd.stream));
                        early_done = true;
                    }
                }
            }
        }
        if (ntap != 4) {
            vda_set_error("vda_forward: the configuration's taps are not four distinct block indices below depth");
            return 1;
        }
        if (!early_done) VDA_TRY(head_early());
        else if (side != nullptr) VDA_HIP(hipStreamWaitEvent(s, side->join, 0));
        void* t3 = act("t3", (size_t)BT * P * ocp[3]);
        VDA_TRY(dense(taps[3], W("proj3.w"), t3, VDA_EPI_BIAS_F16, BT * P, ocp[3], D, V("proj3.b")));
        void* l4 = act("l4", (size_t)BT * h4 * w4 * ocp[3]);
        VDA_TRY(conv3x3(t3, "resize3.w", l4, BT, ph, pw, ocp[3], ocp[3], VDA_EPI_BIAS_F16, 2, V("resize3.b")));
        void* l4t = nullptr;
        VDA_TRY(temporal(1, l4, B, T, h4 * w4, ocp[3], "l4t", &l4t));
        void* l4r = act("l4r", (size_t)BT * h4 * w4 * Fe);
        VDA_TRY(conv3x3(l4t, "rn4.w", l4r, BT, h4, w4, ocp[3], Fe, VDA_EPI_BIAS_F16, 1, nullptr));
        void *p4 = nullptr, *p4t = nullptr, *p3 = nullptr, *p3t = nullptr, *p2 = nullptr, *p1 = nullptr;
        VDA_TRY(fusion(4, l4r, nullptr, BT, h4, w4, ph, pw, Fe, "p4", &p4));
        VDA_TRY(temporal(2, p4, B, T, P, Fe, "p4t", &p4t));
        VDA_TRY(fusion(3, p4t, l3r, BT, ph, pw, h2, w2, Fe, "p3", &p3));
        VDA_TRY(temporal(3, p3, B, T, h2 * w2, Fe, "p3t", &p3t));
        VDA_TRY(fusion(2, p3t, l2r, BT, h2, w2, h1, w1, Fe, "p2", &p2));
        const bool up_fused = prec == VDA_PREC_F16 && h->oc1_fused != 0 && Fhp <= 128 && Fe % 16 == 0;
        VDA_TRY(fusion(1, p2, l1r, BT, h1, w1, 2 * h1, 2 * w1, Fe, up_fused ? "p1c" : "p1", &p1, !up_fused));
        const int hh = 2 * h1, ww = 2 * w1;
        void* o1 = act("o1", (size_t)BT * hh * ww * Fhp);
        if (up_fused) {
            if (!dry) VDA_TRY(vda_conv3x3_up2_f16(p1, W("oc1.w"), V("oc1.b"), o1, BT, h1, w1, Fe, Fhp, Fhp, s));
        } else
            VDA_TRY(conv3x3(p1, "oc1.w", o1, BT, hh, ww, Fe, Fhp, VDA_EPI_BIAS_F16, 1, V("oc1.b")));
        if (prec == VDA_PREC_F16) {
            if (!dry) VDA_TRY(vda_depth_tail_f16(o1, W("oc2.w"), V("oc2.b"), V("oc3.w"), h->oc3_bias, depth, h->zero_page, BT, hh, ww, H, Wd, Fhp, s));
        } else {
            void* up = act("tail_up", (size_t)BT * H * Wd * Fhp);
            VDA_TRY(bilinear(o1, up, BT, hh, ww, H, Wd, Fhp));
            void* c2 = act("tail_c2", (size_t)BT * H * Wd * 32);
            VDA_TRY(conv3x3(up, "oc2.w", c2, BT, H, Wd, Fhp, 32, VDA_EPI_BIAS_RELU_F16, 1, V("oc2.b")));
            if (!dry) VDA_TRY(vda_head_out_f32_f32((const float*)c2, V("oc3.w"), h->oc3_bias, depth, (long long)BT * H * Wd, 32, s));
        }
        if (fold && !dry) {
            hipLaunchKernelGGL(poison_on_overflow_kernel, dim3(256), dim3(256), 0, s, (const int*)ovf, depth, (long long)BT * H * Wd, (volatile int*)h->ovf_host);
            VDA_LAUNCH_CHECK();
        }
        return 0;
    }
};

int get_layout(vda_model* h, int B, int T, int H, int W, int prec, Layout** out) {
    const std::array<int, 5> key = {B, T, H, W, prec};
    auto it = h->layouts.find(key);
    if (it == h->layouts.end()) {
        Layout lay;
        Run r{h, prec, true, &lay, nullptr, prec == VDA_PREC_F32 ? (size_t)4 : (size_t)2};
        VDA_TRY(r.forward(nullptr, nullptr, B, T, H, W));
        lay.gemm_launches = r.nsched;
        size_t off = 0;
        for (const std::string& n : lay.order) {
            lay.bufs[n].first = off;
            off += lay.bufs[n].second;
        }
        lay.total = off;
        it = h->layouts.emplace(key, std::move(lay)).first;
    }
    *out = &it->second;
    return 0;
}

int check_shape(const vda_model* h, int B, int T, int H, int W, int prec) {
    VDA_REQUIRE(prec == VDA_PREC_F16 || prec == VDA_PREC_F32, "vda_forward: precision %d (VDA_PREC_F16 = 0, VDA_PREC_F32 = 1)", prec);
    VDA_REQUIRE(B > 0 && T > 0, "vda_forward: empty clip B=%d T=%d", B, T);
    VDA_REQUIRE(H > 0 && H % PATCH == 0, "Input image height %d is not a multiple of patch height %d", H, PATCH);
    VDA_REQUIRE(W > 0 && W % PATCH == 0, "Input image width %d is not a multiple of patch width: %d", W, PATCH);
    VDA_REQUIRE(T <= h->cfg.num_frames, "vda_forward: T=%d exceeds temporal_max_len=%d", T, h->cfg.num_frames);
    VDA_REQUIRE((long long)B * T * ((H / PATCH) * (W / PATCH) + 1) * 4 * h->cfg.embed_dim < (1ll << 31), "vda_forward: clip too large for 32-bit row offsets (B*T*tokens*4*embed_dim)");
    return 0;
}

}

extern "C" int vda_create(const vda_config* cfg, vda_model** out) {
    VDA_REQUIRE(cfg && out, "vda_create: null argument");
    VDA_REQUIRE(cfg->embed_dim > 0 && cfg->embed_dim % 64 == 0 && cfg->num_heads > 0 && cfg->embed_dim == cfg->num_heads * 64,
                "vda_create: embed_dim=%d must be num_heads=%d x 64 (the attention kernels are built for head dim 64)", cfg->embed_dim, cfg->num_heads);
    VDA_REQUIRE(cfg->depth > 0 && cfg->features > 0 && cfg->features % 64 == 0, "vda_create: depth=%d features=%d (features must be a multiple of 64)", cfg->depth, cfg->features);
    VDA_REQUIRE(cfg->num_frames > 0 && cfg->num_frames <= 32, "vda_create: num_frames=%d must be in 1..32", cfg->num_frames);
    VDA_REQUIRE((cfg->use_clstoken | cfg->use_bn | cfg->pe_rope) >> 1 == 0, "vda_create: use_clstoken / use_bn / pe_rope are 0 or 1");
    for (int i = 0; i < 4; ++i) {
        VDA_REQUIRE(cfg->out_channels[i] > 0 && cfg->out_channels[i] % 8 == 0, "vda_create: out_channels[%d]=%d must be a positive multiple of 8", i, cfg->out_channels[i]);
        VDA_REQUIRE(cfg->taps[i] >= 0 && cfg->taps[i] < cfg->depth && (i == 0 || cfg->taps[i] > cfg->taps[i - 1]), "vda_create: taps must be increasing block indices below depth");
    }
    VDA_REQUIRE(cfg->out_channels[2] % 64 == 0 && cfg->out_channels[3] % 64 == 0,
                "vda_create: out_channels[2..3] carry the temporal modules (GroupNorm over the true width): multiples of 64 only");
    vda_model* h = new vda_model();
    h->cfg = *cfg;
    if (hipGetDevice(&h->device) != hipSuccess) {
        delete h;
        vda_set_error("vda_create: no HIP device (this library has no CPU path)");
        return 2;
    }
    for (int i = 0; i < 4; ++i) h->ocp[i] = pad64(cfg->out_channels[i]);
    h->Fhp = (cfg->features / 2 + 31) / 32 * 32;
    build_spec(h->cfg, h->spec);
    if (dev_alloc(h, 256, &h->zero_page) != 0 || hipMemset(h->zero_page, 0, 256) != hipSuccess) {
        for (void* p : h->owned) (void)hipFree(p);
        delete h;
        vda_set_error("vda_create: device allocation failed");
        return 2;
    }
    void* ring = nullptr;
    if (hipHostMalloc(&ring, 64, hipHostMallocDefault) != hipSuccess) {
        for (void* p : h->owned) (void)hipFree(p);
        delete h;
        vda_set_error("vda_create: pinned host allocation failed");
        return 2;
    }
    memset(ring, 0, 64);
    h->ovf_host = (volatile int32_t*)ring;
    *out = h;
    return 0;
}

extern "C" int vda_destroy(vda_model* h) {
    if (h == nullptr) return 0;
    if (h->ovf_host) (void)hipHostFree((void*)h->ovf_host);
    for (auto& kv : h->sides) {
        if (kv.second.fork) (void)hipEventDestroy(kv.second.fork);
        if (kv.second.join) (void)hipEventDestroy(kv.second.join);
        if (kv.second.stream) (void)hipStreamDestroy(kv.second.stream);
    }
    for (void* p : h->owned) (void)hipFree(p);
    delete h;
    return 0;
}

extern "C" int vda_num_weights(const vda_model* h) { return h ? (int)h->spec.size() : 0; }

static int vda_load_weight_impl(vda_model* h, const char* name, const void* ptr, const int64_t* dims, int ndim, int dtype) {
    VDA_REQUIRE(h && name && ptr && (dims || ndim == 0), "vda_load_weight: null argument");
    VDA_REQUIRE(dtype == VDA_DTYPE_F32, "vda_load_weight(%s): dtype %d (only VDA_DTYPE_F32 = 0 checkpoints are defined, run.py:46)", name, dtype);
    VDA_TRY(require_device(h, "vda_load_weight"));
    auto it = h->spec.find(name);
    VDA_REQUIRE(it != h->spec.end(), "Unexpected key(s) in state_dict: \"%s\". ", name);
    const std::vector<int64_t>& want = it->second;
    bool same = (size_t)ndim == want.size();
    for (int i = 0; same && i < ndim; ++i) same = dims[i] == want[i];
    if (!same) {
        std::string got = "(", exp = "(";
        for (int i = 0; i < ndim; ++i) got += (i ? ", " : "") + std::to_string(dims[i]);
        for (size_t i = 0; i < want.size(); ++i) exp += (i ? ", " : "") + std::to_string(want[i]);
        vda_set_error("size mismatch for %s: copying a param with shape %s) from checkpoint, the shape in current model is %s).", name, got.c_str(), exp.c_str());
        return 1;
    }
    size_t n = 1;
    for (int64_t d : want) n *= (size_t)d;
    Raw& r = h->raw[name];
    if (r.d == nullptr) {
        void* p = nullptr;
        VDA_TRY(dev_alloc(h, n * sizeof(float), &p));
        r.d = (float*)p;
        r.dims = want;
        r.n = n;
    }
    VDA_HIP(hipMemcpy(r.d, ptr, n * sizeof(float), hipMemcpyDefault));
    h->finalized = false;
    return 0;
}

static int vda_finalize_weights_impl(vda_model* h) {
    VDA_REQUIRE(h, "vda_finalize_weights: null handle");
    VDA_TRY(require_device(h, "vda_finalize_weights"));
    std::string missing;
    for (const auto& kv : h->spec)
        if (h->raw.find(kv.first) == h->raw.end()) missing += (missing.empty() ? "\"" : ", \"") + kv.first + "\"";
    if (!missing.empty()) {
        if (missing.size() > 400) missing = missing.substr(0, 400) + " ...";
        vda_set_error("Missing key(s) in state_dict: %s. ", missing.c_str());
        return 1;
    }
    h->mat[0].clear();
    h->mat[1].clear();
    h->vec.clear();
    h->pos_cache.clear();
    h->packed[0] = h->packed[1] = false;
    VDA_HIP(hipMemcpy(&h->oc3_bias, h->raw.at("head.scratch.output_conv2.2.bias").d, sizeof(float), hipMemcpyDeviceToHost));
    VDA_TRY(pack_all<h16>(h, VDA_PREC_F16));
    h->finalized = true;
    return 0;
}

static int vda_prepare_impl(vda_model* h, int B, int T, int H, int W, int precision) {
    VDA_REQUIRE(h && h->finalized, "vda_prepare: load every weight and call vda_finalize_weights first");
    VDA_TRY(require_device(h, "vda_prepare"));
    VDA_TRY(check_shape(h, B, T, H, W, precision));
    if (!h->packed[precision]) VDA_TRY(pack_all<float>(h, VDA_PREC_F32));
    const std::pair<int, int> key = {H, W};
    if (h->pos_cache.find(key) == h->pos_cache.end()) {
        const int ph = H / PATCH, pw = W / PATCH, D = h->cfg.embed_dim;
        const float* pe = h->raw.at("pretrained.pos_embed").d;
        void* p = nullptr;
        VDA_TRY(dev_alloc(h, (size_t)(1 + ph * pw) * D * sizeof(float), &p));
        if (ph * pw == POS_GRID * POS_GRID && H == W) {
            VDA_HIP(hipMemcpyAsync(p, pe, (size_t)(1 + ph * pw) * D * sizeof(float), hipMemcpyDeviceToDevice, nullptr));
        } else {
            VDA_TRY(vda_pos_embed_resample_f32(pe, (float*)p, POS_GRID, ph, pw, D, nullptr));
        }
        VDA_HIP(hipStreamSynchronize(nullptr));
        h->pos_cache[key] = (float*)p;
    }
    Layout* lay = nullptr;
    return get_layout(h, B, T, H, W, precision, &lay);
}

static int64_t vda_workspace_bytes_impl(vda_model* h, int B, int T, int H, int W, int precision) {
    if (h == nullptr || !h->finalized) {
        vda_set_error("vda_workspace_bytes: load every weight and call vda_finalize_weights first");
        return -1;
    }
    if (check_shape(h, B, T, H, W, precision) != 0) return -1;
    Layout* lay = nullptr;
    if (get_layout(h, B, T, H, W, precision, &lay) != 0) return -1;
    return (int64_t)lay->total;
}

extern "C" int vda_set_workspace(vda_model* h, void* ptr, int64_t bytes) {
    VDA_REQUIRE(h, "vda_set_workspace: null handle");
    VDA_REQUIRE(((uintptr_t)ptr & 255) == 0, "vda_set_workspace: the block must be 256-byte aligned");
    h->ws = ptr;
    h->ws_bytes = ptr ? bytes : 0;
    h->ws_owned = false;
    return 0;
}

static int collect_overflow(vda_model* h, const char* who) {
    if (h->ovf_host[0] == 0) return 0;
    h->ovf_host[0] = 0;
    vda_set_error("%s: in a forward since the last check the split residual stream left fp16's range (a token further than 65504 from its own "
                  "mean): that forward's depth was overwritten with NaN. vda_set_option(h, \"ln_fold\", 0) keeps the stream in fp32 (the reference's "
                  "form, no such limit); fp32=True avoids it as well", who);
    return 4;
}

extern "C" int vda_forward_status(vda_model* h) {
    VDA_REQUIRE(h != nullptr, "vda_forward_status: null handle");
    return collect_overflow(h, "vda_forward_status");
}

static int vda_forward_impl(vda_model* h, const float* in, float* out, int B, int T, int H, int W, int precision, vda_stream_t stream) {
    VDA_REQUIRE(h && in && out, "vda_forward: null argument");
    VDA_REQUIRE(h->finalized, "vda_forward: load every weight and call vda_finalize_weights first");
    VDA_TRY(collect_overflow(h, "vda_forward"));
    VDA_TRY(vda_prepare(h, B, T, H, W, precision));
    Layout* lay = nullptr;
    VDA_TRY(get_layout(h, B, T, H, W, precision, &lay));
    if (h->ws == nullptr || (h->ws_owned && (size_t)h->ws_bytes < lay->total)) {
        void* p = nullptr;
        VDA_HIP(hipMalloc(&p, lay->total));
        if (h->ws_owned && h->ws) {
            VDA_HIP(hipDeviceSynchronize());
            (void)hipFree(h->ws);
            for (auto& q : h->owned)
                if (q == h->ws) q = p;
        } else {
            h->owned.push_back(p);
        }
        h->ws = p;
        h->ws_bytes = (int64_t)lay->total;
        h->ws_owned = true;
    }
    VDA_REQUIRE((size_t)h->ws_bytes >= lay->total, "vda_forward: workspace of %lld bytes, this shape needs %lld (vda_workspace_bytes)",
                (long long)h->ws_bytes, (long long)lay->total);
    Run r{h, precision, false, lay, (hipStream_t)stream, precision == VDA_PREC_F32 ? (size_t)4 : (size_t)2};
    h->last_key = {B, T, H, W, precision};
    return r.forward(in, out, B, T, H, W);
}

static int vda_debug_copy_impl(vda_model* h, const char* name, void* dst, int64_t bytes, vda_stream_t stream) {
    VDA_REQUIRE(h && name && dst, "vda_debug_copy: null argument");
    auto it = h->layouts.find(h->last_key);
    VDA_REQUIRE(it != h->layouts.end() && h->ws, "vda_debug_copy: no forward has run");
    auto b = it->second.bufs.find(name);
    VDA_REQUIRE(b != it->second.bufs.end(), "vda_debug_copy: no buffer named %s", name);
    VDA_REQUIRE(bytes > 0 && (size_t)bytes <= b->second.second, "vda_debug_copy: %s holds %lld bytes", name, (long long)b->second.second);
    VDA_HIP(hipMemcpyAsync(dst, (char*)h->ws + b->second.first, (size_t)bytes, hipMemcpyDeviceToDevice, (hipStream_t)stream));
    return 0;
}

extern "C" int vda_set_option(vda_model* h, const char* name, int value) {
    VDA_REQUIRE(h && name, "vda_set_option: null argument");
    if (strcmp(name, "residual_in_ln") == 0) {
        h->residual_in_ln = value;
        h->layouts.clear();
        return 0;
    }
    if (strcmp(name, "profile_min_gflop") == 0) {
        h->prof.min_flops = 1e9 * value;
        return 0;
    }
    if (strcmp(name, "dyn_sched") == 0) {
        h->dyn_sched = value;
        h->layouts.clear();
        return 0;
    }
    if (strcmp(name, "ln_fold") == 0) {
        h->ln_fold = value;
        h->layouts.clear();
        return 0;
    }
    if (strcmp(name, "head_overlap") == 0) {
        h->head_overlap = value != 0;
        return 0;
    }
    if (strcmp(name, "mlp_fused") == 0) {
        h->mlp_fused = value != 0;
        h->layouts.clear();
        return 0;
    }
    if (strcmp(name, "oc1_fused") == 0) {
        h->oc1_fused = value;
        h->layouts.clear();
        return 0;
    }
    vda_set_error("vda_set_option: unknown option %s", name);
    return 1;
}

extern "C" int vda_profile_start(vda_model* h, int every) {
    VDA_REQUIRE(h && every > 0, "vda_profile_start: bad arguments");
    VDA_REQUIRE(h->prof.samples.empty(), "vda_profile_start: a profile is already open");
    const double keep = h->prof.min_flops;
    h->prof = Profile();
    h->prof.every = every;
    h->prof.min_flops = keep;
    return 0;
}

static int vda_profile_stop_impl(vda_model* h, char* json, int cap) {
    VDA_REQUIRE(h && json && cap > 2, "vda_profile_stop: bad arguments");
    Profile& pf = h->prof;
    struct Agg {
        long long timed = 0;
        double ms = 0.0, flops = 0.0;
    };
    std::map<std::string, Agg> agg;
    for (ProfSample& sm : pf.samples) {
        float ms = 0.f;
        hipError_t e = hipEventSynchronize(sm.e1);
        if (e == hipSuccess) e = hipEventElapsedTime(&ms, sm.e0, sm.e1);
        (void)hipEventDestroy(sm.e0);
        (void)hipEventDestroy(sm.e1);
        if (e != hipSuccess) continue;
        Agg& a = agg[sm.name];
        a.timed += 1;
        a.ms += ms;
        a.flops += sm.flops;
    }
    std::string out = "{";
    bool first = true;
    for (const auto& kv : pf.launches) {
        const Agg& a = agg[kv.first];
        char line[512];
        snprintf(line, sizeof(line), "%s\"%s\": {\"launches\": %lld, \"flops\": %.6e, \"timed\": %lld, \"timed_ms\": %.6f, \"timed_flops\": %.6e}",
                 first ? "" : ", ", kv.first.c_str(), kv.second.first, kv.second.second, a.timed, a.ms, a.flops);
        out += line;
        first = false;
    }
    out += "}";
    h->prof = Profile();
    VDA_REQUIRE((int)out.size() + 1 <= cap, "vda_profile_stop: the report needs %d bytes", (int)out.size() + 1);
    memcpy(json, out.c_str(), out.size() + 1);
    return 0;
}

extern "C" int vda_load_weight(vda_model* h, const char* name, const void* ptr, const int64_t* dims, int ndim, int dtype) {
    try {
        return vda_load_weight_impl(h, name, ptr, dims, ndim, dtype);
    } catch (const std::exception& e) {
        vda_set_error("vda_load_weight: %s", e.what());
        return 3;
    }
}

extern "C" int vda_finalize_weights(vda_model* h) {
    try {
        return vda_finalize_weights_impl(h);
    } catch (const std::exception& e) {
        vda_set_error("vda_finalize_weights: %s", e.what());
        return 3;
    }
}

extern "C" int vda_prepare(vda_model* h, int B, int T, int H, int W, int precision) {
    try {
        return vda_prepare_impl(h, B, T, H, W, precision);
    } catch (const std::exception& e) {
        vda_set_error("vda_prepare: %s", e.what());
        return 3;
    }
}

extern "C" int vda_forward(vda_model* h, const float* in, float* out, int B, int T, int H, int W, int precision, vda_stream_t stream) {
    try {
        return vda_forward_impl(h, in, out, B, T, H, W, precision, stream);
    } catch (const std::exception& e) {
        vda_set_error("vda_forward: %s", e.what());
        return 3;
    }
}

extern "C" int vda_debug_copy(vda_model* h, const char* name, void* dst, int64_t bytes, vda_stream_t stream) {
    try {
        return vda_debug_copy_impl(h, name, dst, bytes, stream);
    } catch (const std::exception& e) {
        vda_set_error("vda_debug_copy: %s", e.what());
        return 3;
    }
}

extern "C" int vda_profile_stop(vda_model* h, char* json, int cap) {
    try {
        return vda_profile_stop_impl(h, json, cap);
    } catch (const std::exception& e) {
        vda_set_error("vda_profile_stop: %s", e.what());
        return 3;
    }
}

extern "C" int64_t vda_workspace_bytes(vda_model* h, int B, int T, int H, int W, int precision) {
    try {
        return vda_workspace_bytes_impl(h, B, T, H, W, precision);
    } catch (const std::exception& e) {
        vda_set_error("vda_workspace_bytes: %s", e.what());
        return -1;
    }
}
```

### video_depth_anything_amd/csrc/vda_common.h

```cpp
#pragma once
#include <hip/hip_runtime.h>
#include <hip/hip_fp16.h>
#include <stdint.h>
#include <stdio.h>
#include <stdlib.h>
#include "../../include/vda.h"

typedef _Float16 h16;
typedef _Float16 h16x2 __attribute__((ext_vector_type(2)));
typedef _Float16 h16x4 __attribute__((ext_vector_type(4)));
typedef _Float16 h16x8 __attribute__((ext_vector_type(8)));
typedef float f32x4 __attribute__((ext_vector_type(4)));
typedef float f32x16 __attribute__((ext_vector_type(16)));

#define VDA_GLOBAL_AS __attribute__((address_space(1)))
#define VDA_LDS_AS __attribute__((address_space(3)))

extern "C" void vda_set_error(const char* fmt, ...);

#define VDA_REQUIRE(cond, ...)                 \
    do {                                       \
        if (!(cond)) {                         \
            vda_set_error(__VA_ARGS__);        \
            return 1;                          \
        }                                      \
    } while (0)

#define VDA_LAUNCH_CHECK()                                             \
    do {                                                               \
        hipError_t e_ = hipGetLastError();                             \
        if (e_ != hipSuccess) {                                        \
            vda_set_error("launch failed: %s", hipGetErrorString(e_)); \
            return 2;                                                  \
        }                                                              \
    } while (0)

__device__ __forceinline__ float erf_as(float x) {
    const float ax = fabsf(x);
    const float t = __builtin_amdgcn_rcpf(fmaf(0.3275911f, ax, 1.0f));
    float p = fmaf(1.061405429f, t, -1.453152027f);
    p = fmaf(p, t, 1.421413741f);
    p = fmaf(p, t, -0.284496736f);
    p = fmaf(p, t, 0.254829592f);
    p *= t;
    const float e = __builtin_amdgcn_exp2f(-ax * ax * 1.4426950408889634f);
    const float r = fmaf(-p, e, 1.0f);
    return copysignf(r, x);
}
#define VDA_GELU_C0 1.04427485e+00f
#define VDA_GELU_C1 5.20639309e-02f
#define VDA_GELU_C2 2.21137954e-02f
#define VDA_GELU_C3 3.37046981e-03f
#define VDA_GELU_C4 7.53152628e-05f
#define VDA_GELU_C5 3.96599537e-05f
#define VDA_GELU_C6 6.98591262e-06f
__device__ __forceinline__ float gelu_erf(float x) {
    const float ax = fabsf(x);
    float p = fmaf(VDA_GELU_C6, ax, VDA_GELU_C5);
    p = fmaf(p, ax, VDA_GELU_C4);
    p = fmaf(p, ax, VDA_GELU_C3);
    p = fmaf(p, ax, VDA_GELU_C2);
    p = fmaf(p, ax, VDA_GELU_C1);
    p = fmaf(p, ax, VDA_GELU_C0);
    float r = __builtin_amdgcn_rcpf(p);
    r *= r;
    r *= r;
    r *= r;
    r *= r;
    return fmaf(-ax, r, fmaxf(x, 0.f));
}

typedef float vda_f32x2 __attribute__((ext_vector_type(2)));
__device__ __forceinline__ vda_f32x2 gelu_erf2(vda_f32x2 x) {
    const vda_f32x2 ax = {fabsf(x[0]), fabsf(x[1])};
#define VDA_P2(c) vda_f32x2{c, c}
    vda_f32x2 p = __builtin_elementwise_fma(VDA_P2(VDA_GELU_C6), ax, VDA_P2(VDA_GELU_C5));
    p = __builtin_elementwise_fma(p, ax, VDA_P2(VDA_GELU_C4));
    p = __builtin_elementwise_fma(p, ax, VDA_P2(VDA_GELU_C3));
    p = __builtin_elementwise_fma(p, ax, VDA_P2(VDA_GELU_C2));
    p = __builtin_elementwise_fma(p, ax, VDA_P2(VDA_GELU_C1));
    p = __builtin_elementwise_fma(p, ax, VDA_P2(VDA_GELU_C0));
#undef VDA_P2
    vda_f32x2 r = {__builtin_amdgcn_rcpf(p[0]), __builtin_amdgcn_rcpf(p[1])};
    r *= r;
    r *= r;
    r *= r;
    r *= r;
    const vda_f32x2 relu = {fmaxf(x[0], 0.f), fmaxf(x[1], 0.f)};
    return __builtin_elementwise_fma(-ax, r, relu);
}
template <int N>
__device__ __forceinline__ void gelu_erf_n(float (&v)[N]) {
    static_assert(N % 2 == 0, "pairs");
    constexpr int P = N / 2;
    vda_f32x2 ax[P], p[P], r[P];
#define VDA_P2(c) vda_f32x2{c, c}
#pragma unroll
    for (int k = 0; k < P; ++k) ax[k] = vda_f32x2{fabsf(v[2 * k]), fabsf(v[2 * k + 1])};
#pragma unroll
    for (int k = 0; k < P; ++k) p[k] = __builtin_elementwise_fma(VDA_P2(VDA_GELU_C6), ax[k], VDA_P2(VDA_GELU_C5));
#pragma unroll
    for (int k = 0; k < P; ++k) p[k] = __builtin_elementwise_fma(p[k], ax[k], VDA_P2(VDA_GELU_C4));
#pragma unroll
    for (int k = 0; k < P; ++k) p[k] = __builtin_elementwise_fma(p[k], ax[k], VDA_P2(VDA_GELU_C3));
#pragma unroll
    for (int k = 0; k < P; ++k) p[k] = __builtin_elementwise_fma(p[k], ax[k], VDA_P2(VDA_GELU_C2));
#pragma unroll
    for (int k = 0; k < P; ++k) p[k] = __builtin_elementwise_fma(p[k], ax[k], VDA_P2(VDA_GELU_C1));
#pragma unroll
    for (int k = 0; k < P; ++k) p[k] = __builtin_elementwise_fma(p[k], ax[k], VDA_P2(VDA_GELU_C0));
#undef VDA_P2
#pragma unroll
    for (int k = 0; k < P; ++k) r[k] = vda_f32x2{__builtin_amdgcn_rcpf(p[k][0]), __builtin_amdgcn_rcpf(p[k][1])};
#pragma unroll
    for (int s = 0; s < 4; ++s) {
#pragma unroll
        for (int k = 0; k < P; ++k) r[k] *= r[k];
    }
#pragma unroll
    for (int k = 0; k < P; ++k) {
        const vda_f32x2 relu = {fmaxf(v[2 * k], 0.f), fmaxf(v[2 * k + 1], 0.f)};
        const vda_f32x2 o = __builtin_elementwise_fma(-ax[k], r[k], relu);
        v[2 * k] = o[0];
        v[2 * k + 1] = o[1];
    }
}

__device__ __forceinline__ void glds16(const void* gsrc, void* lds_base) {
    __builtin_amdgcn_global_load_lds((const VDA_GLOBAL_AS void*)gsrc, (VDA_LDS_AS void*)lds_base, 16, 0, 0);
}

__device__ __forceinline__ void glds16_opaque(const void* gsrc, void* lds_base) {
    const unsigned m0v = __builtin_amdgcn_readfirstlane((unsigned)(uintptr_t)lds_base);
    asm volatile("s_mov_b32 m0, %0\n\ts_nop 0\n\tglobal_load_lds_dwordx4 %1, off" ::"s"(m0v), "v"(gsrc) : "memory", "m0");
}

__device__ __forceinline__ float wave_sum(float v) {
#pragma unroll
    for (int o = 32; o > 0; o >>= 1) v += __shfl_xor(v, o, 64);
    return v;
}
__device__ __forceinline__ float wave_max(float v) {
#pragma unroll
    for (int o = 32; o > 0; o >>= 1) v = fmaxf(v, __shfl_xor(v, o, 64));
    return v;
}

__device__ __forceinline__ void load8(const h16* p, float (&v)[8]) {
    const h16x8 x = *reinterpret_cast<const h16x8*>(p);
#pragma unroll
    for (int e = 0; e < 8; ++e) v[e] = (float)x[e];
}
__device__ __forceinline__ void load8(const float* p, float (&v)[8]) {
    const f32x4 a = *reinterpret_cast<const f32x4*>(p), b = *reinterpret_cast<const f32x4*>(p + 4);
#pragma unroll
    for (int e = 0; e < 4; ++e) {
        v[e] = a[e];
        v[4 + e] = b[e];
    }
}
__device__ __forceinline__ void store8(h16* p, const float (&v)[8]) {
    h16x8 o;
#pragma unroll
    for (int e = 0; e < 8; ++e) o[e] = (h16)v[e];
    *reinterpret_cast<h16x8*>(p) = o;
}
__device__ __forceinline__ void store8(float* p, const float (&v)[8]) {
    *reinterpret_cast<f32x4*>(p) = f32x4{v[0], v[1], v[2], v[3]};
    *reinterpret_cast<f32x4*>(p + 4) = f32x4{v[4], v[5], v[6], v[7]};
}

struct VdaKernelDeviceState {
    unsigned long long done = 0;
    int num_cu[64] = {};
};
extern int g_vda_max_wgs;
inline int vda_prepare_kernel(const void* fn, int dyn_lds_bytes, VdaKernelDeviceState& st) {
    int dev = 0;
    (void)hipGetDevice(&dev);
    const int slot = dev & 63;
    if (!((st.done >> slot) & 1ull)) {
        if (dyn_lds_bytes > 48 * 1024) {
            hipError_t e = hipFuncSetAttribute(fn, hipFuncAttributeMaxDynamicSharedMemorySize, dyn_lds_bytes);
            if (e != hipSuccess) {
                vda_set_error("hipFuncSetAttribute: %s", hipGetErrorString(e));
                return -1;
            }
        }
        int cu = 0;
        (void)hipDeviceGetAttribute(&cu, hipDeviceAttributeMultiprocessorCount, dev);
        if (cu < 8) cu = 8;
        st.num_cu[slot] = cu & ~7;
        st.done |= 1ull << slot;
    }
    const int cap = g_vda_max_wgs;
    return (cap >= 8 && cap < st.num_cu[slot]) ? (cap & ~7) : st.num_cu[slot];
}
```

### video_depth_anything_amd/handle.py

```python
import ctypes as C
import json
import os

import torch

from . import _lib
from ._lib import lib
from .config import ModelConfig
from .weights import check_state_dict, state_dict_spec

F16, F32 = torch.float16, torch.float32


def _check(rc, what):
    if rc != 0:
        msg = lib.vda_last_error().decode()
        raise RuntimeError(f"Error(s) in loading state_dict for VideoDepthAnything:\n\t{msg}") if what == "load" else _lib.VdaError(f"{what}: {msg} (rc={rc})")


class ModelHandle:
    def __init__(self, cfg: ModelConfig, device="cuda"):
        if not torch.cuda.is_available():
            raise RuntimeError("video_depth_anything_amd needs an MI355X (HIP device); there is no CPU path")
        self.cfg = cfg
        self.device = torch.device(device)
        if self.device.index is None:
            self.device = torch.device("cuda", torch.cuda.current_device())
        c = _lib.Config(cfg.embed_dim, cfg.depth, cfg.num_heads, (C.c_int32 * 4)(*cfg.taps), cfg.features,
                        (C.c_int32 * 4)(*cfg.out_channels), cfg.num_frames, int(cfg.use_clstoken), int(cfg.use_bn),
                        int(cfg.pe == "rope"))
        h = C.c_void_p()
        with torch.cuda.device(self.device):
            _check(lib.vda_create(C.byref(c), C.byref(h)), "vda_create")
        self._h = h
        self._ws = {}
        if os.environ.get("VDA_RESIDUAL_IN_LN") is not None:
            _check(lib.vda_set_option(h, b"residual_in_ln", int(os.environ["VDA_RESIDUAL_IN_LN"])), "vda_set_option")
        if os.environ.get("VDA_DYN_SCHED") is not None:
            _check(lib.vda_set_option(h, b"dyn_sched", int(os.environ["VDA_DYN_SCHED"])), "vda_set_option")
        if os.environ.get("VDA_HEAD_OVERLAP") is not None:
            _check(lib.vda_set_option(h, b"head_overlap", int(os.environ["VDA_HEAD_OVERLAP"])), "vda_set_option")
        if os.environ.get("VDA_LN_FOLD") is not None:
            _check(lib.vda_set_option(h, b"ln_fold", int(os.environ["VDA_LN_FOLD"])), "vda_set_option")
        self.loaded = False
        assert lib.vda_num_weights(self._h) == len(state_dict_spec(cfg))

    def close(self):
        if getattr(self, "_h", None):
            with torch.cuda.device(self.device):
                torch.cuda.synchronize()
                lib.vda_destroy(self._h)
            self._h = None

    def __del__(self):
        try:
            self.close()
        except Exception:
            pass

    def load_state_dict(self, sd, strict=True):
        check_state_dict(self.cfg, sd, strict)
        spec = state_dict_spec(self.cfg)
        with torch.cuda.device(self.device):
            for name in spec:
                if name not in sd:
                    continue
                t = sd[name].detach()
                if t.dtype != F32 or not t.is_contiguous():
                    t = t.to(F32).contiguous()
                dims = (C.c_int64 * t.dim())(*t.shape)
                _check(lib.vda_load_weight(self._h, name.encode(), C.c_void_p(t.data_ptr()), dims, t.dim(), _lib.DTYPE_F32), "load")
            _check(lib.vda_finalize_weights(self._h), "load")
        self.loaded = True

    def workspace_bytes(self, B, T, H, W, fp32=False):
        n = lib.vda_workspace_bytes(self._h, B, T, H, W, _lib.PREC_F32 if fp32 else _lib.PREC_F16)
        if n < 0:
            raise _lib.VdaError("vda_workspace_bytes: " + lib.vda_last_error().decode())
        return n

    @torch.no_grad()
    def forward(self, x, fp32: bool = False, slot: int = 0):
        if not self.loaded:
            raise RuntimeError("load_state_dict() first")
        if x.dim() != 5 or x.shape[2] != 3:
            raise ValueError(f"expected [B,T,3,H,W], got {tuple(x.shape)}")
        B, T, _, H, W = x.shape
        assert H % 14 == 0, f"Input image height {H} is not a multiple of patch height 14"
        assert W % 14 == 0, f"Input image width {W} is not a multiple of patch width: 14"
        if T > self.cfg.num_frames:
            raise ValueError(f"T={T} exceeds temporal_max_len={self.cfg.num_frames}")
        prec = _lib.PREC_F32 if fp32 else _lib.PREC_F16
        with torch.cuda.device(self.device):
            x = x.to(self.device, F32).contiguous()
            need = self.workspace_bytes(B, T, H, W, fp32)
            ws = self._ws.get(slot)
            if ws is None or ws.numel() < need:
                self._ws[slot] = ws = None
                self._ws[slot] = ws = torch.empty(need, dtype=torch.uint8, device=self.device)
            _check(lib.vda_set_workspace(self._h, C.c_void_p(ws.data_ptr()), ws.numel()), "vda_set_workspace")
            out = torch.empty(B, T, H, W, dtype=F32, device=self.device)
            stream = C.c_void_p(torch.cuda.current_stream(self.device).cuda_stream)
            _check(lib.vda_forward(self._h, C.c_void_p(x.data_ptr()), C.c_void_p(out.data_ptr()), B, T, H, W, prec, stream), "vda_forward")
            self._last = (B * T, H // 14, W // 14, fp32)
        return out

    def check(self, synchronize=True):
        with torch.cuda.device(self.device):
            if synchronize:
                torch.cuda.synchronize(self.device)
            _check(lib.vda_forward_status(self._h), "vda_forward_status")

    def stage(self, name):
        BT, ph, pw, fp32 = self._last
        cfg = self.cfg
        pad = lambda c: (c + 63) // 64 * 64
        oc, Fe = [pad(c) for c in cfg.out_channels], cfg.features
        h4, w4 = (ph - 1) // 2 + 1, (pw - 1) // 2 + 1
        table = {"layer_1": ("l1", 4 * ph, 4 * pw, oc[0]), "layer_2": ("l2", 2 * ph, 2 * pw, oc[1]), "layer_3": ("l3t", ph, pw, oc[2]),
                 "layer_4": ("l4t", h4, w4, oc[3]), "path_4": ("p4t", ph, pw, Fe), "path_3": ("p3t", 2 * ph, 2 * pw, Fe),
                 "path_2": ("p2", 4 * ph, 4 * pw, Fe), "path_1": ("p1", 8 * ph, 8 * pw, Fe)}
        for i in range(4):
            table[f"tap{i}"] = (f"tap{i}", ph, pw, cfg.embed_dim)
        buf, h, w, Cp = table[name]
        t = torch.empty(BT * h * w, Cp, dtype=F32 if fp32 else F16, device=self.device)
        with torch.cuda.device(self.device):
            stream = C.c_void_p(torch.cuda.current_stream(self.device).cuda_stream)
            nbytes = t.numel() * t.element_size()
            if name == "path_1" and lib.vda_debug_copy(self._h, b"p1", C.c_void_p(t.data_ptr()), nbytes, stream) != 0:
                from . import ops
                half = torch.empty(BT * (h // 2) * (w // 2), Cp, dtype=t.dtype, device=self.device)
                _check(lib.vda_debug_copy(self._h, b"p1c", C.c_void_p(half.data_ptr()), half.numel() * half.element_size(), stream), "vda_debug_copy")
                ops.bilinear_nhwc(half, t, BT, h // 2, w // 2, h, w, Cp)
            elif name != "path_1":
                _check(lib.vda_debug_copy(self._h, buf.encode(), C.c_void_p(t.data_ptr()), nbytes, stream), "vda_debug_copy")
        return t, h, w, Cp

    def _check_stage_exists(self, buf):
        probe = torch.empty(16, dtype=torch.uint8, device=self.device)
        with torch.cuda.device(self.device):
            stream = C.c_void_p(torch.cuda.current_stream(self.device).cuda_stream)
            _check(lib.vda_debug_copy(self._h, buf.encode(), C.c_void_p(probe.data_ptr()), 16, stream), "vda_debug_copy")

    def set_option(self, name, value):
        _check(lib.vda_set_option(self._h, name.encode(), int(value)), "vda_set_option")

    def profile_start(self, every=4):
        _check(lib.vda_profile_start(self._h, every), "vda_profile_start")

    def profile_stop(self):
        buf = C.create_string_buffer(1 << 16)
        with torch.cuda.device(self.device):
            _check(lib.vda_profile_stop(self._h, buf, len(buf)), "vda_profile_stop")
        return json.loads(buf.value.decode())
```

### video_depth_anything_amd/video_depth.py

```python
import numpy as np
import torch

from .config import INFER_LEN, get_config
from .scheduler import network_size


def _all_gather(out, inp):
    import torch.distributed as dist
    if dist.get_backend() == "nccl":
        return dist.all_gather_into_tensor(out, inp, async_op=True)
    parts = [torch.empty(inp.shape, dtype=inp.dtype) for _ in range(dist.get_world_size())]
    dist.all_gather(parts, inp.cpu())
    out.copy_(torch.stack(parts))
    return None


class VideoDepthAnything:
    METRIC = False

    def __init__(self, encoder='vits', features=64, out_channels=[48, 96, 192, 384], use_bn=False, use_clstoken=False,
                 num_frames=32, pe='ape', **_unused):
        self.encoder = encoder
        self.intermediate_layer_idx = {'vits': [2, 5, 8, 11], 'vitl': [4, 11, 17, 23]}
        self.cfg = get_config(encoder, features, out_channels, num_frames, use_clstoken, use_bn, pe)
        self.engine = None
        self._device = torch.device('cuda' if torch.cuda.is_available() else 'cpu')
        self._sd = None
        self.result_ranks = None
        self.exchange = "windows"

    def load_state_dict(self, state_dict, strict=True):
        from .weights import check_state_dict
        check_state_dict(self.cfg, state_dict, strict)
        self._sd = state_dict
        if self.engine is not None:
            self.engine.load_state_dict(state_dict, strict)
        return self

    def to(self, device):
        device = torch.device(device)
        if device.type != 'cuda':
            raise RuntimeError("video_depth_anything_amd runs on an MI355X HIP device only (got device=%r)" % (device,))
        if device.index is None:
            device = torch.device('cuda', torch.cuda.current_device())
        if self.engine is not None and device != self.engine.device:
            self.engine.close()
            self.engine = None
        self._device = device
        self._ensure_engine()
        return self

    def cuda(self):
        return self.to('cuda')

    def eval(self):
        return self

    def _ensure_engine(self):
        if self.engine is None:
            from .handle import ModelHandle
            self.engine = ModelHandle(self.cfg, self._device)
            if self._sd is not None:
                self.engine.load_state_dict(self._sd, True)
        return self.engine

    def python_engine(self):
        from .engine import Engine
        if self.cfg.use_bn or self.cfg.pe != "ape":
            raise NotImplementedError("the Python launch sequence (engine.py) covers the released configurations only; "
                                      "use_bn / pe='rope' run through the handle (vda_forward)")
        e = Engine(self.cfg, self._ensure_engine().device)
        e.load_state_dict(self._sd, True)
        return e

    def forward(self, x, fp32=None):
        if fp32 is None:
            fp32 = not torch.is_autocast_enabled()
        return self._ensure_engine().forward(x, fp32=bool(fp32))

    __call__ = forward

    def infer_video_depth(self, frames, target_fps, input_size=518, device='cuda', fp32=False):
        if torch.device(device).type != 'cuda':
            raise RuntimeError("video_depth_anything_amd runs on an MI355X HIP device only (got device=%r)" % (device,))
        eng = self._ensure_engine()
        with torch.cuda.device(eng.device):
            return self._infer_video_depth(eng, frames, target_fps, input_size, bool(fp32))

    def _infer_video_depth(self, eng, frames, target_fps, input_size, fp32):
        import torch.distributed as dist
        from . import ops
        from .scheduler import drive_windows, plan_windows, shard_windows
        from .stitch import stitch_stream
        if not isinstance(frames, np.ndarray):
            frames = np.asarray(frames)
        if frames.ndim != 4 or frames.shape[-1] != 3:
            raise ValueError("infer_video_depth: frames must be [N, H, W, 3], got shape %r" % (tuple(frames.shape),))
        if frames.dtype != np.uint8:
            ok = True
            for i in range(0, frames.shape[0], 64):
                c = np.asarray(frames[i:i + 64])
                ok = bool(c.size == 0 or (c.min() >= 0 and c.max() <= 255 and
                                          (np.issubdtype(c.dtype, np.integer) or np.array_equal(c, np.rint(c)))))
                if not ok:
                    break
            if not ok:
                raise TypeError("infer_video_depth: frames must hold 8-bit values (uint8, or any dtype whose values are integers "
                                "within 0..255); got dtype %s with other values" % frames.dtype)
            frames = frames.astype(np.uint8)
        H0, W0 = frames.shape[1:3]
        H, W = network_size(H0, W0, input_size)
        dev = eng.device
        n = frames.shape[0]
        plan = plan_windows(n)
        world = dist.get_world_size() if (dist.is_available() and dist.is_initialized()) else 1
        rank = dist.get_rank() if world > 1 else 0
        mine = list(shard_windows(len(plan), world, rank))
        eng.set_option("dyn_sched", 1 if world > 1 else 0)

        need = sorted({f for k in mine for f in plan[k]})
        slot_of = {f: i for i, f in enumerate(need)}
        video = torch.empty((max(len(need), 1), H0, W0, 3), dtype=torch.uint8, device=dev)
        compute = torch.cuda.current_stream(dev)
        upload = torch.cuda.Stream(device=dev)
        resident = set()

        def ensure(k):
            if k is None:
                return
            todo = sorted(f for f in set(plan[k]) if f not in resident)
            with torch.cuda.stream(upload):
                i = 0
                while i < len(todo):
                    j = i
                    while j + 1 < len(todo) and todo[j + 1] == todo[j] + 1:
                        j += 1
                    s0 = slot_of[todo[i]]
                    run = frames[todo[i]:todo[j] + 1]
                    if not (run.flags.c_contiguous and run.flags.writeable):
                        run = np.array(run)
                    video[s0:s0 + (j - i + 1)].copy_(torch.from_numpy(run), non_blocking=True)
                    i = j + 1
            resident.update(todo)

        NSLOT = 2
        lanes = [torch.cuda.Stream(device=dev) for _ in range(NSLOT)]
        computed = [torch.cuda.Event() for _ in range(NSLOT)]
        freed = [torch.cuda.Event() for _ in range(NSLOT)]
        xin = [torch.empty(1, INFER_LEN, 3, H, W, dtype=torch.float32, device=dev) for _ in range(NSLOT)]
        send = [torch.empty(INFER_LEN, H0, W0, dtype=torch.float32, device=dev) for _ in range(NSLOT)]
        recv = [torch.empty(world, INFER_LEN, H0, W0, dtype=torch.float32, device=dev) for _ in range(NSLOT)] if world > 1 else None
        used = [False] * NSLOT

        def acquire(s):
            if used[s]:
                lanes[s].wait_event(freed[s])
            used[s] = True

        def window_depth(k, s, keys=None):
            ensure(k)
            lane = lanes[s]
            lane.wait_stream(upload)
            acquire(s)
            with torch.cuda.stream(lane):
                idx = torch.tensor([slot_of[f] for f in plan[k]], dtype=torch.int32, device=dev)
                if (H0, W0) == (H, W):
                    ops.gather_normalize_u8(video, idx, xin[s], INFER_LEN, H0, W0)
                else:
                    ops.gather_resize_normalize_u8(video, idx, xin[s], INFER_LEN, H0, W0, H, W)
                depth = eng.forward(xin[s], fp32=fp32, slot=s)
                ops.bilinear_plane(depth.view(INFER_LEN, H, W), send[s], INFER_LEN, H, W, H0, W0)
                if keys is not None:
                    keys[0:2].copy_(send[s][0:2])
                    keys[2].copy_(send[s][12])
                    keys[3:].copy_(send[s][INFER_LEN - 8:])
                computed[s].record(lane)
            pos = mine.index(k)
            ensure(mine[pos + 1] if pos + 1 < len(mine) else None)

        def exchange(s):
            acquire(s)
            with torch.cuda.stream(lanes[s]):
                h = _all_gather(recv[s], send[s])
                if h is not None:
                    h.wait()
                computed[s].record(lanes[s])
            return None

        def ready(s):
            compute.wait_event(computed[s])

        def release(s):
            freed[s].record(compute)

        if self.exchange == "keys":
            from .scheduler import KEY_SLOTS, drive_windows_keys
            from .stitch import DeviceKeyOps, collect_pieces
            assert tuple(KEY_SLOTS) == (0, 1, 12) + tuple(range(INFER_LEN - 8, INFER_LEN))

            def gather_keys(s, out, inp):
                acquire(s)
                with torch.cuda.stream(lanes[s]):
                    if world > 1:
                        h = _all_gather(out, inp)
                        if h is not None:
                            h.wait()
                    else:
                        out[0].copy_(inp)
                    computed[s].record(lanes[s])
                return None

            kops = DeviceKeyOps(send, H0, W0, dev, self.METRIC, world, rank, len(plan), self.result_ranks, window_depth, ready, release,
                                gather_keys, acquire)
            pieces = drive_windows_keys(len(plan), world, rank, kops, self.result_ranks)
            if self.result_ranks is not None and rank not in self.result_ranks:
                for _ in pieces:
                    pass
                eng.check()
                return None, target_fps
            depths = collect_pieces(pieces, n, H0, W0, dev, on_copied=kops.copied)
            for lane in lanes:
                compute.wait_stream(lane)
            eng.check()
            return depths, target_fps

        windows = drive_windows(len(plan), world, rank, send, recv, window_depth, exchange, ready, release)
        if self.result_ranks is not None and rank not in self.result_ranks:
            for _ in windows:
                pass
            eng.check()
            return None, target_fps
        depths = stitch_stream(windows, n, H0, W0, dev, metric=self.METRIC)
        for lane in lanes:
            compute.wait_stream(lane)
        eng.check()
        return depths, target_fps


class MetricVideoDepthAnything(VideoDepthAnything):
    METRIC = True

    def __init__(self, encoder='vitl', features=256, out_channels=[256, 512, 1024, 1024], use_bn=False, use_clstoken=False,
                 num_frames=32, pe='ape'):
        super().__init__(encoder, features, out_channels, use_bn, use_clstoken, num_frames, pe)
```

Before: 626.8 frames/s.

## Split encoder into two frame halves on parallel streams to overlap blocks

Splits the ViT encoder's per-block work (LN-folded GEMMs, attention, residual GEMMs, tap layernorms, readout) into two halves of the frames, issuing the second half on a separate lane stream so the two halves can run concurrently on the GPU. A planned-M hint is passed to the GEMM dispatcher so tile selection still uses the full row count instead of the half. The aim is to fill idle compute units between dependent kernels and hide the tails of small launches. In exchange it adds fork/join events, halves the per-launch work, and turns the split off during graph capture, when other streams have pending work, and in infer_video_depth.

```diff
diff --git a/video_depth_anything_amd/csrc/gemm.hip b/video_depth_anything_amd/csrc/gemm.hip
--- a/video_depth_anything_amd/csrc/gemm.hip
+++ b/video_depth_anything_amd/csrc/gemm.hip
@@ -314,11 +314,13 @@
     return 0;
 }
 
-static int vda_gemm_f16_impl(const vda_gemm_args* args, vda_stream_t stream, bool may_split);
-
-extern "C" int vda_gemm_f16(const vda_gemm_args* args, vda_stream_t stream) { return vda_gemm_f16_impl(args, stream, true); }
-
-static int vda_gemm_f16_impl(const vda_gemm_args* args, vda_stream_t stream, bool may_split) {
+static int vda_gemm_f16_impl(const vda_gemm_args* args, vda_stream_t stream, bool may_split, int m_plan);
+
+extern "C" int vda_gemm_f16(const vda_gemm_args* args, vda_stream_t stream) { return vda_gemm_f16_impl(args, stream, true, 0); }
+
+int vda_gemm_f16_planned(const vda_gemm_args* args, vda_stream_t stream, int m_plan) { return vda_gemm_f16_impl(args, stream, true, m_plan); }
+
+static int vda_gemm_f16_impl(const vda_gemm_args* args, vda_stream_t stream, bool may_split, int m_plan) {
     VDA_REQUIRE(args != nullptr, "vda_gemm_f16: null args");
     vda_gemm_args a = *args;
     VDA_REQUIRE(a.A && a.W && a.out, "vda_gemm_f16: null operand");
@@ -383,6 +385,7 @@
             break;
     }
     hipStream_t s = (hipStream_t)stream;
+    const int Mp = m_plan > a.M ? m_plan : a.M;
     static const int conv_lds = getenv("VDA_CONV_LDS") ? atoi(getenv("VDA_CONV_LDS")) : 1;
     if (a.a_mode == VDA_A_CONV3X3 && ((g_gemm_variant < 0 && conv_lds) || g_gemm_variant == 7)) {
         const int rc = vda_conv3x3_lds(a, s);
@@ -405,7 +408,7 @@
         big = 128;
     }
     static const int big_min_n = getenv("VDA_GEMM_BIG_MIN_N") ? atoi(getenv("VDA_GEMM_BIG_MIN_N")) : 192;
-    if (g_gemm_variant < 0 && a.N >= big_min_n && a.M >= 2048) {
+    if (g_gemm_variant < 0 && a.N >= big_min_n && Mp >= 2048) {
         const int pad256 = (a.N + 255) / 256 * 256, pad128 = (a.N + 127) / 128 * 128;
         big = pad128 < pad256 ? 128 : 256;
         static const int eight128 = getenv("VDA_GEMM_8P128") ? atoi(getenv("VDA_GEMM_8P128")) : 0;
@@ -423,18 +426,18 @@
         if (eight && g_gemm_variant > 0) a8.relu_in = (a.relu_in & 0xff) | (((g_gemm_variant >> 4) & 0xff) << 8);
         a8.relu_in |= g_gemm_debug << 16;
         static const long long nt_mb = getenv("VDA_GEMM_NT_MB") ? atoll(getenv("VDA_GEMM_NT_MB")) : 192;
-        if (nt_mb > 0 && (long long)a.M * a.N * 2 >= nt_mb * 1000000ll) a8.relu_in |= 1 << 24;
+        if (nt_mb > 0 && (long long)Mp * a.N * 2 >= nt_mb * 1000000ll) a8.relu_in |= 1 << 24;
         const int sched8 = (eight && g_gemm_variant > 0) ? ((g_gemm_variant >> 5) & 3) : 0;
         bool tall192 = g_gemm_variant == 8 && a.a_mode == VDA_A_DENSE;
         const int ncu = device_cus();
         if (g_gemm_variant < 0 && !eight && big == 128 && a.a_mode == VDA_A_DENSE) {
             const long long nbn = (a.N + 127) / 128;
-            const long long r256 = (((a.M + 255) / 256) * nbn + ncu - 1) / ncu, r192 = (((a.M + 191) / 192) * nbn + ncu - 1) / ncu;
+            const long long r256 = (((Mp + 255) / 256) * nbn + ncu - 1) / ncu, r192 = (((Mp + 191) / 192) * nbn + ncu - 1) / ncu;
             static const int allow192 = getenv("VDA_GEMM_BM192") ? atoi(getenv("VDA_GEMM_BM192")) : 1;
             tall192 = allow192 && r192 * 3 * 100 < r256 * 4 * 85;
         }
         static const int small_grid = getenv("VDA_GEMM_SMALL_GRID") ? atoi(getenv("VDA_GEMM_SMALL_GRID")) : 1;
-        if (g_gemm_variant < 0 && small_grid && ((long long)(a.M + 255) / 256) * ((a.N + big - 1) / big) * 2 <= ncu) {
+        if (g_gemm_variant < 0 && small_grid && ((long long)(Mp + 255) / 256) * ((a.N + big - 1) / big) * 2 <= ncu) {
             g_last_kernel = a.a_mode == VDA_A_DENSE ? (a.N <= 64 ? "gemm_kernel<128, 64, 0>" : "gemm_kernel<128, 128, 0>")
                                                     : (a.N <= 64 ? "gemm_kernel<128, 64, 1>" : "gemm_kernel<128, 128, 1>");
             return launch_small(a, s);
@@ -455,14 +458,15 @@
                 return rc384;
             }
         }
-        if (eight && big == 256 && a.a_mode == VDA_A_DENSE && g_gemm_variant < 0 && may_split && a.tile_rows == 0 && a.sched == nullptr && a.lda != 0) {
+        if (eight && big == 256 && a.a_mode == VDA_A_DENSE && g_gemm_variant < 0 && may_split && Mp == a.M && a.tile_rows == 0 && a.sched == nullptr &&
+            a.lda != 0) {
             const int m1 = vda_gemm_plan_split(a.M, a.N, a.K, a.epilogue, a.a_mode);
             if (m1 < a.M) {
                 vda_gemm_args p1 = row_range(a, 0, m1), p2 = row_range(a, m1, a.M - m1);
                 p2.tile_rows = 192;
-                const int rc1 = vda_gemm_f16_impl(&p1, stream, false);
+                const int rc1 = vda_gemm_f16_impl(&p1, stream, false, m_plan);
                 if (rc1 != 0) return rc1;
-                return vda_gemm_f16_impl(&p2, stream, false);
+                return vda_gemm_f16_impl(&p2, stream, false, m_plan);
             }
         }
         if (eight && big == 256 && a.a_mode == VDA_A_DENSE && (a.tile_rows == 192 || g_gemm_variant == 5 + 16 * 64)) {
diff --git a/video_depth_anything_amd/csrc/host.hip b/video_depth_anything_amd/csrc/host.hip
--- a/video_depth_anything_amd/csrc/host.hip
+++ b/video_depth_anything_amd/csrc/host.hip
@@ -150,6 +150,9 @@
         hipEvent_t fork = nullptr, join = nullptr;
     };
     std::map<hipStream_t, Side> sides;
+    int enc_split = 1;
+    std::map<hipStream_t, Side> lanes;
+    std::map<hipStream_t, hipEvent_t> tails;
     int mlp_fused = 0;
     volatile int32_t* ovf_host = nullptr;
 };
@@ -494,6 +497,7 @@
     size_t ab;
     int32_t* sched = nullptr;
     int nsched = 0;
+    int mplan = 0;
 
     void* buf(const std::string& name, size_t elems, size_t esize) {
         const size_t bytes = (elems * esize + 255) & ~(size_t)255;
@@ -515,7 +519,7 @@
     const float* V(const std::string& k) const { return dry ? nullptr : h->vec.at(k); }
 
     int gemm(vda_gemm_args a) {
-        if (prec == VDA_PREC_F16) {
+        if (prec == VDA_PREC_F16 && mplan == 0) {
             const int m1 = vda_gemm_plan_split(a.M, a.N, a.K, a.epilogue, a.a_mode);
             if (m1 < a.M) {
                 if (dry) {
@@ -544,7 +548,7 @@
         if (a.lda == 0) a.lda = a.K;
         if (a.ldc == 0) a.ldc = a.N;
         Profile& pf = h->prof;
-        if (pf.every <= 0) return prec == VDA_PREC_F32 ? vda_gemm_f32(&a, s) : vda_gemm_f16(&a, s);
+        if (pf.every <= 0) return prec == VDA_PREC_F32 ? vda_gemm_f32(&a, s) : vda_gemm_f16_planned(&a, s, mplan);
         const std::array<int, 5> key = {a.M, a.N, a.K, a.epilogue, a.a_mode};
         const int n = pf.seen[key]++;
         const bool timed = n % pf.every == 0 && 2.0 * a.M * a.N * a.K >= pf.min_flops;
@@ -554,7 +558,7 @@
             VDA_HIP(hipEventCreate(&smp.e1));
             VDA_HIP(hipEventRecord(smp.e0, s));
         }
-        VDA_TRY(prec == VDA_PREC_F32 ? vda_gemm_f32(&a, s) : vda_gemm_f16(&a, s));
+        VDA_TRY(prec == VDA_PREC_F32 ? vda_gemm_f32(&a, s) : vda_gemm_f16_planned(&a, s, mplan));
         const std::string name = prec == VDA_PREC_F32 ? std::string("gemm_f32_kernel") : std::string(vda_gemm_last_kernel());
         const double flops = 2.0 * a.M * a.N * a.K;
         auto& tot = pf.launches[name];
@@ -672,6 +676,15 @@
         const vda_config& c = h->cfg;
         const int BT = B * T, ph = H / PATCH, pw = Wd / PATCH;
         const int P = ph * pw, D = c.embed_dim, NH = c.num_heads, Nt = P + 1, rows = BT * Nt;
+        bool capturing = false;
+        if (!dry) {
+            hipStreamCaptureStatus cs = hipStreamCaptureStatusNone;
+            if (hipStreamIsCapturing(s, &cs) != hipSuccess) {
+                (void)hipGetLastError();
+                cs = hipStreamCaptureStatusActive;
+            }
+            capturing = cs != hipStreamCaptureStatusNone;
+        }
         if (prec == VDA_PREC_F16 && h->dyn_sched) {
             const int cap = dry ? 4096 : lay->gemm_launches;
             sched = (int32_t*)buf("sched", (size_t)8 * (cap > 0 ? cap : 1), 4);
@@ -709,27 +722,87 @@
         int32_t* ovf = fold ? (int32_t*)buf("overflow", 1, 4) : nullptr;
         if (fold && !dry) VDA_HIP(hipMemsetAsync(ovf, 0, 4, s));
         if (fold && !dry) VDA_TRY(vda_split_center_stats_f32(tok, thi, tlo, lnstat, ENC_LN_EPS, rows, D, s));
-        auto ln_gemm = [&](const std::string& wk, void* out, int epi, int N) -> int {
+        struct Part {
+            int f0, nf;
+            hipStream_t st;
+        };
+        Part parts[2] = {{0, BT, s}, {0, 0, nullptr}};
+        int nparts = 1;
+        vda_model::Side* lane = nullptr;
+        bool split = fold && !mlp1 && h->enc_split != 0 && BT >= 2;
+        if (split && !dry) {
+            split = !capturing;
+            for (auto& kv : h->tails) {
+                if (!split) break;
+                if (kv.first == s || kv.second == nullptr) continue;
+                if (hipEventQuery(kv.second) != hipSuccess) {
+                    (void)hipGetLastError();
+                    split = false;
+                }
+            }
+        }
+        if (split) {
+            parts[0] = {0, BT / 2, s};
+            parts[1] = {BT / 2, BT - BT / 2, s};
+            nparts = 2;
+            if (!dry) {
+                vda_model::Side& ln = h->lanes[s];
+                if (ln.stream == nullptr) {
+                    VDA_HIP(hipStreamCreateWithFlags(&ln.stream, hipStreamNonBlocking));
+                    VDA_HIP(hipEventCreateWithFlags(&ln.fork, hipEventDisableTiming));
+                    VDA_HIP(hipEventCreateWithFlags(&ln.join, hipEventDisableTiming));
+                }
+                lane = &ln;
+                parts[1].st = ln.stream;
+                VDA_HIP(hipEventRecord(ln.fork, s));
+                VDA_HIP(hipStreamWaitEvent(ln.stream, ln.fork, 0));
+            }
+        }
+        auto each = [&](auto&& fn) -> int {
+            const hipStream_t keep = s;
+            int rc = 0;
+            for (int j = 0; j < nparts && rc == 0; ++j) {
+                s = parts[j].st;
+                rc = fn(parts[j]);
+            }
+            s = keep;
+            return rc;
+        };
+        auto ln_gemm = [&](const std::string& wk, void* out, int epi, int N, const Part& p) -> int {
+            const size_t r0 = (size_t)p.f0 * Nt;
             vda_gemm_args a = {};
-            a.A = thi, a.W = W(wk + ".weight.ln"), a.out = out, a.bias = V(wk + ".c2"), a.gamma = V(wk + ".c1"), a.stats = lnstat;
-            a.M = rows, a.N = N, a.K = D, a.a_mode = VDA_A_DENSE, a.epilogue = epi;
-            return gemm(a);
+            a.A = (const h16*)thi + r0 * D, a.W = W(wk + ".weight.ln"), a.out = (h16*)out + r0 * N, a.bias = V(wk + ".c2"), a.gamma = V(wk + ".c1");
+            a.stats = lnstat + r0 * 2;
+            a.M = p.nf * Nt, a.N = N, a.K = D, a.a_mode = VDA_A_DENSE, a.epilogue = epi;
+            mplan = nparts > 1 ? rows : 0;
+            const int rc = gemm(a);
+            mplan = 0;
+            return rc;
         };
-        auto res_gemm = [&](const void* A, const std::string& wk, const std::string& gk, int K, bool stats_next) -> int {
+        auto res_gemm = [&](const void* A, const std::string& wk, const std::string& gk, int K, bool stats_next, const Part& p) -> int {
+            const size_t r0 = (size_t)p.f0 * Nt;
+            const int nr = p.nf * Nt, np = D / 64;
             vda_gemm_args a = {};
-            a.A = A, a.W = W(wk + ".weight"), a.out = thi, a.out2 = tlo, a.res = thi, a.res2 = tlo, a.bias = V(wk + ".bias"), a.gamma = V(gk);
-            a.stats = lnpart;
-            a.pos = lnstat;
-            a.M = rows, a.N = D, a.K = K, a.a_mode = VDA_A_DENSE, a.epilogue = VDA_EPI_SCALE_RES_SPLIT;
-            VDA_TRY(gemm(a));
+            a.A = (const h16*)A + r0 * K, a.W = W(wk + ".weight"), a.bias = V(wk + ".bias"), a.gamma = V(gk);
+            a.out = (h16*)thi + r0 * D, a.out2 = (h16*)tlo + r0 * D, a.res = a.out, a.res2 = a.out2;
+            a.stats = lnpart + r0 * np * 2;
+            a.pos = lnstat + r0 * 2;
+            a.M = nr, a.N = D, a.K = K, a.a_mode = VDA_A_DENSE, a.epilogue = VDA_EPI_SCALE_RES_SPLIT;
+            mplan = nparts > 1 ? rows : 0;
+            const int rc = gemm(a);
+            mplan = 0;
+            VDA_TRY(rc);
             (void)stats_next;
-            if (!dry) VDA_TRY(vda_ln_stats_finalize(lnpart, lnstat, ENC_LN_EPS, rows, D / 64, ovf, s));
+            if (!dry) VDA_TRY(vda_ln_stats_finalize(lnpart + r0 * np * 2, lnstat + r0 * 2, ENC_LN_EPS, nr, np, ovf, s));
             return 0;
         };
-        auto tap_ln = [&](void* out, int group, int skip) -> int {
+        auto tap_ln = [&](void* out, int group, int skip, const Part& p) -> int {
             if (dry) return 0;
-            return fold ? vda_layernorm_split_f16(thi, tlo, out, V("norm.w"), V("norm.b"), ENC_LN_EPS, rows, D, group, skip, s)
-                        : vda_layernorm_f32_f16(tok, out, V("norm.w"), V("norm.b"), ENC_LN_EPS, rows, D, group, skip, nullptr, 0, 0, s);
+            const size_t r0 = (size_t)p.f0 * Nt, o0 = group > 0 ? (size_t)p.f0 * (Nt / group) * (group - skip) : r0;
+            const int nr = p.nf * Nt;
+            return fold ? vda_layernorm_split_f16((const h16*)thi + r0 * D, (const h16*)tlo + r0 * D, (h16*)out + o0 * D, V("norm.w"), V("norm.b"), ENC_LN_EPS, nr, D,
+                                                  group, skip, s)
+                        : vda_layernorm_f32_f16(tok + r0 * D, (h16*)out + o0 * D, V("norm.w"), V("norm.b"), ENC_LN_EPS, nr, D, group, skip, nullptr, 0, 0, s);
         };
         void* yb = defer ? act("ybuf", (size_t)rows * D) : nullptr;
         auto ln_res = [&](const float* gamma, void* out, const float* w, const float* b, int group, int skip) -> int {
@@ -779,15 +852,20 @@
         for (int i = 0; i < c.depth; ++i) {
             const std::string k = "b" + std::to_string(i) + ".";
             if (fold) {
-                VDA_TRY(ln_gemm(k + "attn.qkv", qkv, VDA_EPI_LN_BIAS_F16, 3 * D));
+                VDA_TRY(each([&](const Part& p) { return ln_gemm(k + "attn.qkv", qkv, VDA_EPI_LN_BIAS_F16, 3 * D, p); }));
             } else {
                 if (!xn_ready) VDA_TRY(layernorm(tok, xn, V(k + "norm1.weight"), V(k + "norm1.bias"), ENC_LN_EPS, rows, D));
                 xn_ready = false;
                 VDA_TRY(dense(xn, W(k + "attn.qkv.weight"), qkv, VDA_EPI_BIAS_F16, rows, 3 * D, D, V(k + "attn.qkv.bias")));
             }
-            if (!dry) VDA_TRY(prec == VDA_PREC_F32 ? vda_attention_f32((const float*)qkv, (float*)ao, BT, Nt, NH, s) : vda_attention_f16(qkv, ao, BT, Nt, NH, s));
+            if (!dry)
+                VDA_TRY(each([&](const Part& p) {
+                    const size_t r0 = (size_t)p.f0 * Nt;
+                    return prec == VDA_PREC_F32 ? vda_attention_f32((const float*)qkv + r0 * 3 * D, (float*)ao + r0 * D, p.nf, Nt, NH, s)
+                                                : vda_attention_f16((const h16*)qkv + r0 * 3 * D, (h16*)ao + r0 * D, p.nf, Nt, NH, s);
+                }));
             if (fold) {
-                VDA_TRY(res_gemm(ao, k + "attn.proj", k + "ls1.gamma", D, true));
+                VDA_TRY(each([&](const Part& p) { return res_gemm(ao, k + "attn.proj", k + "ls1.gamma", D, true, p); }));
             } else if (defer) {
                 VDA_TRY(dense(ao, W(k + "attn.proj.weight"), yb, VDA_EPI_BIAS_F16, rows, D, D, V(k + "attn.proj.bias")));
                 VDA_TRY(ln_res(V(k + "ls1.gamma"), xn, V(k + "norm2.weight"), V(k + "norm2.bias"), 0, 0));
@@ -799,7 +877,7 @@
                 if (!dry)
                     VDA_TRY(vda_mlp_fused_f16(thi, lnstat, W(k + "mlp.fc1.weight.ln"), V(k + "mlp.fc1.c1"), V(k + "mlp.fc1.c2"), W(k + "mlp.fc2.weight.perm"),
                                               V(k + "mlp.fc2.bias"), V(k + "ls2.gamma"), thi, tlo, lnpart, rows, D, 4 * D, rows, s));
-            } else if (fold) VDA_TRY(ln_gemm(k + "mlp.fc1", hid, VDA_EPI_LN_GELU_F16, 4 * D));
+            } else if (fold) VDA_TRY(each([&](const Part& p) { return ln_gemm(k + "mlp.fc1", hid, VDA_EPI_LN_GELU_F16, 4 * D, p); }));
             else VDA_TRY(dense(xn, W(k + "mlp.fc1.weight"), hid, VDA_EPI_BIAS_GELU_F16, rows, 4 * D, D, V(k + "mlp.fc1.bias")));
             bool is_tap = false;
             for (int t = 0; t < 4; ++t) is_tap = is_tap || c.taps[t] == i;
@@ -809,9 +887,9 @@
                 if (mlp1) {
                     if (!dry) VDA_TRY(vda_ln_stats_finalize(lnpart, lnstat, ENC_LN_EPS, rows, D / 64, ovf, s));
                 } else {
-                    VDA_TRY(res_gemm(hid, k + "mlp.fc2", k + "ls2.gamma", 4 * D, !last));
+                    VDA_TRY(each([&](const Part& p) { return res_gemm(hid, k + "mlp.fc2", k + "ls2.gamma", 4 * D, !last, p); }));
                 }
-                if (tp != nullptr) VDA_TRY(tap_ln(tp, Nt, 1));
+                if (tp != nullptr) VDA_TRY(each([&](const Part& p) { return tap_ln(tp, Nt, 1, p); }));
             } else if (defer) {
                 VDA_TRY(dense(hid, W(k + "mlp.fc2.weight"), yb, VDA_EPI_BIAS_F16, rows, D, 4 * D, V(k + "mlp.fc2.bias")));
                 if (last && tp != nullptr) {
@@ -829,13 +907,20 @@
             if (tp != nullptr) {
                 if (c.use_clstoken) {
                     void* full = act("rd_full", (size_t)rows * D);
-                    VDA_TRY(fold ? tap_ln(full, 0, 0) : layernorm(tok, full, V("norm.w"), V("norm.b"), ENC_LN_EPS, rows, D));
                     void* cat = act("rd_cat", (size_t)BT * P * 2 * D);
-                    if (!dry)
-                        VDA_TRY(prec == VDA_PREC_F32 ? vda_readout_concat_f32((const float*)full, (float*)cat, BT, P, D, s)
-                                                     : vda_readout_concat_f16(full, cat, BT, P, D, s));
                     const std::string kr = "readout" + std::to_string(ntap);
-                    VDA_TRY(dense(cat, W(kr + ".w"), tp, VDA_EPI_BIAS_GELU_F16, BT * P, D, 2 * D, V(kr + ".b")));
+                    VDA_TRY(each([&](const Part& p) -> int {
+                        const size_t r0 = (size_t)p.f0 * Nt, q0 = (size_t)p.f0 * P;
+                        VDA_TRY(fold ? tap_ln(full, 0, 0, p) : layernorm(tok, full, V("norm.w"), V("norm.b"), ENC_LN_EPS, rows, D));
+                        if (!dry)
+                            VDA_TRY(prec == VDA_PREC_F32 ? vda_readout_concat_f32((const float*)full + r0 * D, (float*)cat + q0 * 2 * D, p.nf, P, D, s)
+                                                         : vda_readout_concat_f16((const h16*)full + r0 * D, (h16*)cat + q0 * 2 * D, p.nf, P, D, s));
+                        mplan = nparts > 1 ? BT * P : 0;
+                        const int rc = dense((const char*)cat + q0 * 2 * D * ab, W(kr + ".w"), (char*)tp + q0 * D * ab, VDA_EPI_BIAS_GELU_F16, p.nf * P, D, 2 * D,
+                                             V(kr + ".b"));
+                        mplan = 0;
+                        return rc;
+                    }));
                 }
                 taps[ntap++] = tp;
                 if (ntap == 3 && !last && !early_done) {
@@ -854,6 +939,10 @@
                         side = &sd;
                         VDA_HIP(hipEventRecord(sd.fork, s));
                         VDA_HIP(hipStreamWaitEvent(sd.stream, sd.fork, 0));
+                        if (lane != nullptr) {
+                            VDA_HIP(hipEventRecord(lane->join, lane->stream));
+                            VDA_HIP(hipStreamWaitEvent(sd.stream, lane->join, 0));
+                        }
                         hipStream_t main_stream = s;
                         s = sd.stream;
                         const int rc = head_early();
@@ -864,6 +953,10 @@
                     }
                 }
             }
+        }
+        if (lane != nullptr) {
+            VDA_HIP(hipEventRecord(lane->join, lane->stream));
+            VDA_HIP(hipStreamWaitEvent(s, lane->join, 0));
         }
         if (ntap != 4) {
             vda_set_error("vda_forward: the configuration's taps are not four distinct block indices below depth");
@@ -906,6 +999,11 @@
             hipLaunchKernelGGL(poison_on_overflow_kernel, dim3(256), dim3(256), 0, s, (const int*)ovf, depth, (long long)BT * H * Wd, (volatile int*)h->ovf_host);
             VDA_LAUNCH_CHECK();
         }
+        if (!dry && !capturing) {
+            hipEvent_t& tail = h->tails[s];
+            if (tail == nullptr) VDA_HIP(hipEventCreateWithFlags(&tail, hipEventDisableTiming));
+            VDA_HIP(hipEventRecord(tail, s));
+        }
         return 0;
     }
 };
@@ -940,6 +1038,11 @@
     return 0;
 }
 
+int enc_split_default() {
+    static const int v = getenv("VDA_ENC_SPLIT") ? atoi(getenv("VDA_ENC_SPLIT")) : 1;
+    return v != 0;
+}
+
 }
 
 extern "C" int vda_create(const vda_config* cfg, vda_model** out) {
@@ -980,6 +1083,7 @@
     }
     memset(ring, 0, 64);
     h->ovf_host = (volatile int32_t*)ring;
+    h->enc_split = enc_split_default();
     *out = h;
     return 0;
 }
@@ -987,11 +1091,14 @@
 extern "C" int vda_destroy(vda_model* h) {
     if (h == nullptr) return 0;
     if (h->ovf_host) (void)hipHostFree((void*)h->ovf_host);
-    for (auto& kv : h->sides) {
-        if (kv.second.fork) (void)hipEventDestroy(kv.second.fork);
-        if (kv.second.join) (void)hipEventDestroy(kv.second.join);
-        if (kv.second.stream) (void)hipStreamDestroy(kv.second.stream);
-    }
+    for (auto& kv : h->tails)
+        if (kv.second) (void)hipEventDestroy(kv.second);
+    for (auto* m : {&h->sides, &h->lanes})
+        for (auto& kv : *m) {
+            if (kv.second.fork) (void)hipEventDestroy(kv.second.fork);
+            if (kv.second.join) (void)hipEventDestroy(kv.second.join);
+            if (kv.second.stream) (void)hipStreamDestroy(kv.second.stream);
+        }
     for (void* p : h->owned) (void)hipFree(p);
     delete h;
     return 0;
@@ -1172,6 +1279,11 @@
     }
     if (strcmp(name, "head_overlap") == 0) {
         h->head_overlap = value != 0;
+        return 0;
+    }
+    if (strcmp(name, "enc_split") == 0) {
+        h->enc_split = value < 0 ? enc_split_default() : value != 0;
+        h->layouts.clear();
         return 0;
     }
     if (strcmp(name, "mlp_fused") == 0) {
diff --git a/video_depth_anything_amd/csrc/vda_common.h b/video_depth_anything_amd/csrc/vda_common.h
--- a/video_depth_anything_amd/csrc/vda_common.h
+++ b/video_depth_anything_amd/csrc/vda_common.h
@@ -175,6 +175,7 @@
     int num_cu[64] = {};
 };
 extern int g_vda_max_wgs;
+int vda_gemm_f16_planned(const vda_gemm_args* args, vda_stream_t stream, int m_plan);
 inline int vda_prepare_kernel(const void* fn, int dyn_lds_bytes, VdaKernelDeviceState& st) {
     int dev = 0;
     (void)hipGetDevice(&dev);
diff --git a/video_depth_anything_amd/handle.py b/video_depth_anything_amd/handle.py
--- a/video_depth_anything_amd/handle.py
+++ b/video_depth_anything_amd/handle.py
@@ -34,6 +34,7 @@
             _check(lib.vda_create(C.byref(c), C.byref(h)), "vda_create")
         self._h = h
         self._ws = {}
+        self.options = {}
         if os.environ.get("VDA_RESIDUAL_IN_LN") is not None:
             _check(lib.vda_set_option(h, b"residual_in_ln", int(os.environ["VDA_RESIDUAL_IN_LN"])), "vda_set_option")
         if os.environ.get("VDA_DYN_SCHED") is not None:
@@ -144,6 +145,7 @@
 
     def set_option(self, name, value):
         _check(lib.vda_set_option(self._h, name.encode(), int(value)), "vda_set_option")
+        self.options[name] = int(value)
 
     def profile_start(self, every=4):
         _check(lib.vda_profile_start(self._h, every), "vda_profile_start")
diff --git a/video_depth_anything_amd/video_depth.py b/video_depth_anything_amd/video_depth.py
--- a/video_depth_anything_amd/video_depth.py
+++ b/video_depth_anything_amd/video_depth.py
@@ -84,8 +84,13 @@
         if torch.device(device).type != 'cuda':
             raise RuntimeError("video_depth_anything_amd runs on an MI355X HIP device only (got device=%r)" % (device,))
         eng = self._ensure_engine()
-        with torch.cuda.device(eng.device):
-            return self._infer_video_depth(eng, frames, target_fps, input_size, bool(fp32))
+        keep = eng.options.get("enc_split", -1)
+        eng.set_option("enc_split", 0)
+        try:
+            with torch.cuda.device(eng.device):
+                return self._infer_video_depth(eng, frames, target_fps, input_size, bool(fp32))
+        finally:
+            eng.set_option("enc_split", keep)
 
     def _infer_video_depth(self, eng, frames, target_fps, input_size, fp32):
         import torch.distributed as dist
```

Measured after the change: 639.9 frames/s (median of 6 runs). 1.02x the previous value.
